# haan6/fm-for-online-recommendation

Measured on NVIDIA B200. Metric: train samples/sec (fwd+bwd+update), higher is better.
Workload: dtype f32

## Files before the change

### fm_for_online_recommendation_b200/csrc/radix_sort.cu

```cuda
#include "fmb_common.cuh"
#include "smem_sort.cuh"
#include <cooperative_groups.h>
namespace cg = cooperative_groups;

namespace {

constexpr int RADIX_BITS = 8;
constexpr int CL_SEGS = 4;
__device__ long long* g_sort_dbg = nullptr;
__device__ __forceinline__ void sort_stamp(int slot) {
    if (g_sort_dbg && threadIdx.x == 0) { unsigned long long gt; asm volatile("mov.u64 %0, %globaltimer;" : "=l"(gt)); g_sort_dbg[slot] = (long long)gt; }
}
constexpr int RADIX = 1 << RADIX_BITS;
constexpr int SORT_THREADS = 256;
constexpr int SORT_WARPS = SORT_THREADS / 32;
constexpr int KPT = 8;
constexpr int TILE = SORT_THREADS * KPT;

__device__ __forceinline__ int digit_of(int32_t key, int shift) { return (key >> shift) & (RADIX - 1); }

using fmb::digit_peers;

__global__ void __launch_bounds__(SORT_THREADS) radix_hist_kernel(const int32_t* __restrict__ keys, int64_t N,
                                                                  int shift, int ntiles,
                                                                  uint32_t* __restrict__ hist) {
    __shared__ uint32_t h[RADIX];
    for (int i = threadIdx.x; i < RADIX; i += SORT_THREADS) h[i] = 0;
    __syncthreads();
    const int64_t base = (int64_t)blockIdx.x * TILE;
#pragma unroll
    for (int i = 0; i < KPT; ++i) {
        const int64_t idx = base + (int64_t)i * SORT_THREADS + threadIdx.x;
        if (idx < N) atomicAdd(&h[digit_of(keys[idx], shift)], 1u);
    }
    __syncthreads();
    for (int i = threadIdx.x; i < RADIX; i += SORT_THREADS) hist[(size_t)i * ntiles + blockIdx.x] = h[i];
}

__global__ void __launch_bounds__(256) radix_scan_rows_kernel(uint32_t* __restrict__ hist, int ntiles, uint32_t* __restrict__ rowtot) {
    __shared__ uint32_t warp_tot[8];
    __shared__ uint32_t carry_s;
    const int lane = threadIdx.x & 31, warp = threadIdx.x >> 5;
    uint32_t* row = hist + (size_t)blockIdx.x * ntiles;
    if (threadIdx.x == 0) carry_s = 0;
    __syncthreads();
    constexpr int IPT = 4;
    for (int base = 0; base < ntiles; base += 256 * IPT) {
        const int i0 = base + threadIdx.x * IPT;
        uint32_t v[IPT], sum = 0;
#pragma unroll
        for (int j = 0; j < IPT; ++j) { v[j] = (i0 + j < ntiles) ? row[i0 + j] : 0u; sum += v[j]; }
        uint32_t inc = sum;
#pragma unroll
        for (int o = 1; o < 32; o <<= 1) { uint32_t t = __shfl_up_sync(0xffffffffu, inc, o); if (lane >= o) inc += t; }
        if (lane == 31) warp_tot[warp] = inc;
        __syncthreads();
        uint32_t before = 0, all = 0;
#pragma unroll
        for (int w = 0; w < 8; ++w) { const uint32_t t = warp_tot[w]; if (w < warp) before += t; all += t; }
        const uint32_t carry = carry_s;
        uint32_t excl = carry + before + (inc - sum);
#pragma unroll
        for (int j = 0; j < IPT; ++j) { if (i0 + j < ntiles) row[i0 + j] = excl; excl += v[j]; }
        __syncthreads();
        if (threadIdx.x == 0) carry_s = carry + all;
        __syncthreads();
    }
    if (threadIdx.x == 0) rowtot[blockIdx.x] = carry_s;
}

__global__ void __launch_bounds__(SORT_THREADS) radix_scatter_kernel(const int32_t* __restrict__ keys_in,
                                                                     const int32_t* __restrict__ vals_in, int64_t N,
                                                                     int shift, int ntiles,
                                                                     const uint32_t* __restrict__ scan,
                                                                     const uint32_t* __restrict__ rowtot,
                                                                     int32_t* __restrict__ keys_out,
                                                                     int32_t* __restrict__ vals_out) {
    __shared__ uint32_t cnt[SORT_WARPS][RADIX];
    __shared__ uint32_t gbase[RADIX];
    const int lane = threadIdx.x & 31, warp = threadIdx.x >> 5;
    for (int i = threadIdx.x; i < SORT_WARPS * RADIX; i += SORT_THREADS) (&cnt[0][0])[i] = 0;
    for (int i = threadIdx.x; i < RADIX; i += SORT_THREADS) gbase[i] = scan[(size_t)i * ntiles + blockIdx.x];
    __syncthreads();
    if (warp == 0) {
        uint32_t v[8], sum = 0;
#pragma unroll
        for (int j = 0; j < 8; ++j) { v[j] = rowtot[lane * 8 + j]; sum += v[j]; }
        uint32_t inc = sum;
#pragma unroll
        for (int o = 1; o < 32; o <<= 1) { const uint32_t t = __shfl_up_sync(0xffffffffu, inc, o); if (lane >= o) inc += t; }
        uint32_t ex = inc - sum;
#pragma unroll
        for (int j = 0; j < 8; ++j) { gbase[lane * 8 + j] += ex; ex += v[j]; }
    }
    __syncthreads();
    const int64_t wbase = (int64_t)blockIdx.x * TILE + (int64_t)warp * 32 * KPT;
    int32_t key[KPT];
    uint32_t rank[KPT];
    const uint32_t lt = (1u << lane) - 1u;
#pragma unroll
    for (int i = 0; i < KPT; ++i) {
        const int64_t idx = wbase + i * 32 + lane;
        const bool valid = idx < N;
        key[i] = valid ? keys_in[idx] : 0;
        const unsigned d = valid ? (unsigned)digit_of(key[i], shift) : 0u;
        const unsigned m = digit_peers(d, valid);
        const int leader = __ffs(m) - 1;
        uint32_t old = 0;
        if (valid && lane == leader) { old = cnt[warp][d]; cnt[warp][d] = old + __popc(m); }
        old = __shfl_sync(0xffffffffu, old, leader);
        rank[i] = old + __popc(m & lt);
        __syncwarp();
    }
    __syncthreads();
    for (int d = threadIdx.x; d < RADIX; d += SORT_THREADS) {
        uint32_t run = 0;
#pragma unroll
        for (int w = 0; w < SORT_WARPS; ++w) { uint32_t t = cnt[w][d]; cnt[w][d] = run; run += t; }
    }
    __syncthreads();
#pragma unroll
    for (int i = 0; i < KPT; ++i) {
        const int64_t idx = wbase + i * 32 + lane;
        if (idx < N) {
            const int d = digit_of(key[i], shift);
            const uint32_t pos = gbase[d] + cnt[warp][d] + rank[i];
            keys_out[pos] = key[i];
            vals_out[pos] = vals_in ? vals_in[idx] : (int32_t)idx;
        }
    }
}

__global__ void __launch_bounds__(1024) segment_starts_kernel(const int32_t* __restrict__ keys, int64_t N,
                                                              int32_t* __restrict__ seg_start,
                                                              int32_t* __restrict__ nseg) {
    __shared__ uint32_t warp_tot[32];
    __shared__ uint32_t carry_s;
    const int lane = threadIdx.x & 31, warp = threadIdx.x >> 5;
    if (threadIdx.x == 0) carry_s = 0;
    __syncthreads();
    for (int64_t base = 0; base < N; base += 1024) {
        const int64_t i = base + threadIdx.x;
        const uint32_t f = (i < N) && (i == 0 || keys[i] != keys[i - 1]);
        uint32_t inc = f;
#pragma unroll
        for (int o = 1; o < 32; o <<= 1) { uint32_t t = __shfl_up_sync(0xffffffffu, inc, o); if (lane >= o) inc += t; }
        if (lane == 31) warp_tot[warp] = inc;
        __syncthreads();
        if (warp == 0) {
            uint32_t w = warp_tot[lane], winc = w;
#pragma unroll
            for (int o = 1; o < 32; o <<= 1) { uint32_t t = __shfl_up_sync(0xffffffffu, winc, o); if (lane >= o) winc += t; }
            warp_tot[lane] = winc - w;
        }
        __syncthreads();
        const uint32_t pos = carry_s + warp_tot[warp] + inc - f;
        if (f) seg_start[pos] = (int32_t)i;
        __syncthreads();
        if (threadIdx.x == 1023) carry_s = pos + f;
        __syncthreads();
    }
    if (threadIdx.x == 0) { *nseg = (int32_t)carry_s; seg_start[carry_s] = (int32_t)N; }
}



template <int THREADS, typename KeyAt>
__device__ __forceinline__ void sort_tail(const uint32_t* kc, const uint16_t* pc, int n, int g0, int B, int F, int f,
                                          int32_t off, int32_t* __restrict__ skeys, int32_t* __restrict__ perm,
                                          uint32_t* __restrict__ posflag, int4* __restrict__ rl_entries,
                                          uint32_t* __restrict__ rl_segc, int rl_cap, int rl_nseg, int seg, int seg_long, KeyAt key_at) {
    __shared__ uint32_t wcount_s[32], wcountl_s[32];
    const int lane = threadIdx.x & 31, warp = threadIdx.x >> 5;
    const uint32_t lt = (1u << lane) - 1u;
    const int nr = (n + 31) & ~31;
    int4* mine = rl_entries ? rl_entries + (size_t)seg * rl_cap : nullptr;
    int4* minel = rl_entries ? rl_entries + (size_t)seg_long * rl_cap : nullptr;
    auto is_long = [&](int i, uint32_t key) {
        const int g2 = g0 + i + 127, j2 = i + 127;
        return g2 < B && (j2 < n ? kc[j2] : key_at(g2)) == key;
    };
    uint32_t wc = 0, wcl = 0;
    for (int i = threadIdx.x; i < nr; i += THREADS) {
        bool start = false, lng = false;
        if (i < n) {
            const int gi = g0 + i;
            const uint32_t key = kc[i];
            const uint32_t prev = gi > 0 ? (i > 0 ? kc[i - 1] : key_at(gi - 1)) : 0xffffffffu;
            const uint32_t next = gi + 1 < B ? (i + 1 < n ? kc[i + 1] : key_at(gi + 1)) : 0xffffffffu;
            const bool cont = key == prev, multi = cont || key == next;
            start = multi && !cont;
            if (start && mine) lng = is_long(i, key);
            const size_t o = (size_t)f * B + gi;
            const int32_t e = (int32_t)pc[i] * F + f;
            skeys[o] = (int32_t)key + off;
            perm[o] = e;
            if (posflag) posflag[e] = (uint32_t)o | (multi ? 0x80000000u : 0u);
        }
        if (mine) {
            wc += __popc(__ballot_sync(0xffffffffu, start && !lng));
            wcl += __popc(__ballot_sync(0xffffffffu, lng));
        }
    }
    if (!mine) return;
    if (lane == 0) { wcount_s[warp] = wc; wcountl_s[warp] = wcl; }
    __syncthreads();
    uint32_t base = 0, total = 0, basel = 0, totall = 0;
    for (int w = 0; w < THREADS / 32; ++w) {
        const uint32_t t = wcount_s[w], tl = wcountl_s[w];
        if (w < warp) { base += t; basel += tl; }
        total += t; totall += tl;
    }
    if (threadIdx.x == 0) { rl_segc[seg] = total; rl_segc[rl_nseg + seg_long] = totall; }
    if (wc + wcl == 0) return;
    for (int i = threadIdx.x; i < nr; i += THREADS) {
        uint32_t key = 0xfffffffeu;
        bool cont = false, start = false, lng = false;
        const int gi = g0 + i;
        if (i < n) {
            key = kc[i];
            const uint32_t prev = gi > 0 ? (i > 0 ? kc[i - 1] : key_at(gi - 1)) : 0xffffffffu;
            const uint32_t next = gi + 1 < B ? (i + 1 < n ? kc[i + 1] : key_at(gi + 1)) : 0xffffffffu;
            cont = key == prev;
            start = !cont && key == next;
            if (start) lng = is_long(i, key);
        }
        const unsigned m = __ballot_sync(0xffffffffu, start);
        if (m) {
            const unsigned ml = __ballot_sync(0xffffffffu, lng);
            const unsigned cm = __ballot_sync(0xffffffffu, cont);
            const uint32_t klast = __shfl_sync(0xffffffffu, key, 31);
            const int i2 = i + 32, gi2 = gi + 32;
            const uint32_t k2 = gi2 < B ? (i2 < n ? kc[i2] : key_at(gi2)) : 0xffffffffu;
            const unsigned em = __ballot_sync(0xffffffffu, k2 == klast);
            const int ext = em == 0xffffffffu ? 32 : __ffs(~em) - 1;
            if (start) {
                const unsigned after = lane == 31 ? 0u : (cm >> (lane + 1));
                const int inw = lane == 31 ? 0 : __ffs(~after) - 1;
                int n0 = 1 + inw;
                if (lane + inw == 31) n0 += ext;
                if (n0 > 32) n0 = 32;
                const int4 e4 = make_int4((int)((size_t)f * B + gi), (int32_t)key + off, n0, lng ? 1 : 0);
                if (lng) minel[rl_cap - 1 - (int)(basel + __popc(ml & lt))] = e4;
                else mine[base + __popc((m & ~ml) & lt)] = e4;
            }
            base += __popc(m & ~ml);
            basel += __popc(ml);
        }
    }
}

constexpr int SPARSE_THREADS = 1024;
constexpr int SPARSE_DIRECT = 256;

__host__ __device__ inline int sparse_table_slots(int B) { int t = 1024; while (t < 2 * B) t <<= 1; return t; }
__host__ __device__ inline size_t sparse_region_bytes(int B) {
    const size_t a = (size_t)sparse_table_slots(B) * 4, b = (size_t)B * 4 + (size_t)(B + (B & 1)) * 2 + 32 * 256 * 2;
    return a > b ? a : b;
}
__host__ __device__ inline int sparse_bp(int B) { return B < 2048 ? 2048 : B; }
__host__ __device__ inline size_t sparse_smem_bytes(int B) {
    return (size_t)B * 4 + (size_t)((B + 3) & ~3) + (size_t)sparse_bp(B) * 4 + (size_t)((sparse_bp(B) + 1) & ~1) * 2 + sparse_region_bytes(B) + 16;
}

__global__ void __launch_bounds__(SPARSE_THREADS) sparse_fields_kernel(const int32_t* __restrict__ ids, int B, int F,
                                                                      const int32_t* __restrict__ field_off,
                                                                      int64_t min_rows, int32_t* __restrict__ skeys,
                                                                      int32_t* __restrict__ perm, uint32_t* __restrict__ posflag,
                                                                      int4* __restrict__ rl_entries, uint32_t* __restrict__ rl_segc,
                                                                      int rl_cap) {
    const int f = blockIdx.x;
    const int32_t off = field_off[f];
    const uint32_t nrows = (uint32_t)(field_off[f + 1] - off);
    if ((int64_t)nrows < min_rows) return;
    extern __shared__ __align__(16) unsigned char sp_smem[];
    const int slots = sparse_table_slots(B);
    uint32_t* keys = reinterpret_cast<uint32_t*>(sp_smem);
    uint8_t* flag = reinterpret_cast<uint8_t*>(keys + B);
    const int Bp = sparse_bp(B);
    uint32_t* kbuf0 = reinterpret_cast<uint32_t*>(flag + ((B + 3) & ~3));
    uint16_t* pbuf0 = reinterpret_cast<uint16_t*>(kbuf0 + Bp);
    uint32_t* tab = reinterpret_cast<uint32_t*>(pbuf0 + ((Bp + 1) & ~1));
    uint32_t* kbuf1 = tab;
    uint16_t* pbuf1 = reinterpret_cast<uint16_t*>(kbuf1 + B);
    uint16_t* cnt = pbuf1 + B + (B & 1);
    __shared__ uint32_t tot[256];
    __shared__ uint32_t wsum[32];
    __shared__ uint32_t nm_s, t_fill, t_filll;
    const int lane = threadIdx.x & 31, warp = threadIdx.x >> 5;
    const uint32_t lt = (1u << lane) - 1u;
    sort_stamp(16 + 2 * F + 2 * f);
    for (int i0 = threadIdx.x; i0 < B; i0 += 8 * SPARSE_THREADS) {
        int32_t v[8];
#pragma unroll
        for (int u = 0; u < 8; ++u) { const int i = i0 + u * SPARSE_THREADS; v[u] = i < B ? __ldg(ids + (size_t)i * F + f) : 0; }
#pragma unroll
        for (int u = 0; u < 8; ++u) {
            const int i = i0 + u * SPARSE_THREADS;
            if (i < B) { keys[i] = (uint32_t)(v[u] - off); flag[i] = 0; }
        }
    }
    for (int i = threadIdx.x; i < slots; i += SPARSE_THREADS) tab[i] = 0;
    if (threadIdx.x == 0) { t_fill = 0; t_filll = 0; }
    __syncthreads();
    sort_stamp(16 + 6 * F + f);
    {
        constexpr int PER = 8;
        const uint32_t mask = (uint32_t)slots - 1u;
        const int hshift = 32 - (31 - __clz(slots));
        uint32_t key[PER], slot[PER], step[PER];
        unsigned open = 0;
#pragma unroll
        for (int u = 0; u < PER; ++u) {
            const int i = threadIdx.x + u * SPARSE_THREADS;
            key[u] = 0; slot[u] = 0; step[u] = 1;
            if (i < B) {
                key[u] = keys[i];
                slot[u] = (key[u] * 2654435761u) >> hshift;
                step[u] = ((key[u] * 0x85ebca6bu) >> 17) | 1u;
                open |= 1u << u;
            }
        }
#pragma unroll
        for (int u = 0; u < PER; ++u)
            if ((open >> u) & 1u) { if (tab[slot[u]] == 0u) tab[slot[u]] = (uint32_t)(threadIdx.x + u * SPARSE_THREADS) + 1u; }
        __syncthreads();
        const int perb = (B + SPARSE_THREADS - 1) / SPARSE_THREADS;
        uint16_t* ulist = reinterpret_cast<uint16_t*>(kbuf0) + warp * (perb * 32);
        uint16_t* uslot = ulist + SPARSE_THREADS * perb;
        int wn = 0;
#pragma unroll
        for (int u = 0; u < PER; ++u) {
            bool unsettled = false;
            const uint32_t me = (uint32_t)(threadIdx.x + u * SPARSE_THREADS) + 1u;
            if ((open >> u) & 1u) {
                const uint32_t cur = tab[slot[u]];
                if (cur == me) { }
                else if (keys[cur - 1] == key[u]) { flag[cur - 1] = 1; flag[me - 1] = 1; }
                else unsettled = true;
            }
            const unsigned um = __ballot_sync(0xffffffffu, unsettled);
            if (unsettled) {
                const int j = wn + __popc(um & lt);
                ulist[j] = (uint16_t)(me - 1u);
                uslot[j] = (uint16_t)((slot[u] + step[u]) & mask);
            }
            wn += __popc(um);
        }
        __syncthreads();
        for (int j = lane; j < wn; j += 32) {
            const uint32_t i = ulist[j], k = keys[i];
            const uint32_t st = ((k * 0x85ebca6bu) >> 17) | 1u;
            uint32_t sl = uslot[j];
            for (;;) {
                const uint32_t old = atomicCAS(&tab[sl], 0u, i + 1u);
                if (old == 0u) break;
                if (keys[old - 1] == k) { flag[old - 1] = 1; flag[i] = 1; break; }
                sl = (sl + st) & mask;
            }
        }
    }
    __syncthreads();
    sort_stamp(16 + 7 * F + f);
    const int per = (B + SPARSE_THREADS - 1) / SPARSE_THREADS;
    const int i0 = threadIdx.x * per;
    uint32_t mine = 0;
    for (int u = 0; u < per; ++u) if (i0 + u < B) mine += flag[i0 + u];
    uint32_t inc = mine;
#pragma unroll
    for (int o = 1; o < 32; o <<= 1) { const uint32_t t = __shfl_up_sync(0xffffffffu, inc, o); if (lane >= o) inc += t; }
    if (lane == 31) wsum[warp] = inc;
    __syncthreads();
    if (warp == 0) {
        const uint32_t w = wsum[lane];
        uint32_t winc = w;
#pragma unroll
        for (int o = 1; o < 32; o <<= 1) { const uint32_t t = __shfl_up_sync(0xffffffffu, winc, o); if (lane >= o) winc += t; }
        wsum[lane] = winc - w;
        if (lane == 31) nm_s = winc;
    }
    __syncthreads();
    {
        uint32_t o = wsum[warp] + inc - mine;
        for (int u = 0; u < per; ++u)
            if (i0 + u < B && flag[i0 + u]) { kbuf0[o] = keys[i0 + u]; pbuf0[o] = (uint16_t)(i0 + u); ++o; }
    }
    __syncthreads();
    const int nm = (int)nm_s;
    sort_stamp(16 + 5 * F + f);
    uint32_t* ks = kbuf1;
    uint16_t* ps = pbuf1;
    if (nm <= SPARSE_DIRECT) {
        for (int a = threadIdx.x; a < nm; a += SPARSE_THREADS) {
            const uint32_t key = kbuf0[a];
            int r = 0;
            for (int b2 = 0; b2 < nm; ++b2) { const uint32_t kb = kbuf0[b2]; r += (kb < key) || (kb == key && b2 < a); }
            kbuf1[r] = key;
            pbuf1[r] = pbuf0[a];
        }
        __syncthreads();
    } else {
        const int bits = nrows <= 1 ? 0 : 32 - __clz(nrows - 1);
        fmb::smem_sort_passes(kbuf0, kbuf1, pbuf0, pbuf1, cnt, tot, nm, (bits + RADIX_BITS - 1) / RADIX_BITS, &ks, &ps);
    }
    sort_stamp(16 + 8 * F + f);
    const size_t fb = (size_t)f * B;
    for (int i = nm + threadIdx.x; i < B; i += SPARSE_THREADS) skeys[fb + i] = -1;
    int4* seg = rl_entries ? rl_entries + (size_t)(f * CL_SEGS) * rl_cap : nullptr;
    const int nr = (nm + 31) & ~31;
    for (int a = threadIdx.x; a < nr; a += SPARSE_THREADS) {
        bool start = false;
        uint32_t key = 0;
        if (a < nm) {
            key = ks[a];
            const int32_t e = (int32_t)ps[a] * F + f;
            skeys[fb + a] = (int32_t)key + off;
            perm[fb + a] = e;
            posflag[e] = (uint32_t)(fb + a) | 0x80000000u;
            start = a == 0 || ks[a - 1] != key;
        }
        if (seg && start) {
            int n0 = 1;
            while (n0 < 32 && a + n0 < nm && ks[a + n0] == key) ++n0;
            const bool lng = a + 127 < nm && ks[a + 127] == key;
            const int4 e4 = make_int4((int)(fb + a), (int32_t)key + off, n0, lng ? 1 : 0);
            if (lng) seg[CL_SEGS * rl_cap - 1 - (int)atomicAdd(&t_filll, 1u)] = e4;
            else seg[atomicAdd(&t_fill, 1u)] = e4;
        }
    }
    if (seg) {
        __syncthreads();
        if (threadIdx.x < CL_SEGS) {
            rl_segc[f * CL_SEGS + threadIdx.x] = threadIdx.x == 0 ? t_fill : 0u;
            rl_segc[F * CL_SEGS + f * CL_SEGS + threadIdx.x] = threadIdx.x == CL_SEGS - 1 ? t_filll : 0u;
        }
    }
    sort_stamp(17 + 2 * F + 2 * f);
}

constexpr int FS_THREADS = 1024;
constexpr int FS_WARPS = FS_THREADS / 32;
constexpr int FS_MAX_SLOTS = 16;

__global__ void __launch_bounds__(FS_THREADS) sort_fields_kernel(const int32_t* __restrict__ ids, int B, int F,
                                                                 const int32_t* __restrict__ field_off,
                                                                 int32_t* __restrict__ skeys,
                                                                 int32_t* __restrict__ perm, uint32_t* __restrict__ posflag,
                                                                 int4* __restrict__ rl_entries, uint32_t* __restrict__ rl_segc,
                                                                 int rl_cap, int64_t max_rows) {
    extern __shared__ __align__(16) unsigned char fs_smem[];
    uint32_t* kbuf0 = reinterpret_cast<uint32_t*>(fs_smem);
    uint32_t* kbuf1 = kbuf0 + B;
    uint16_t* pbuf0 = reinterpret_cast<uint16_t*>(kbuf1 + B);
    uint16_t* pbuf1 = pbuf0 + B + (B & 1);
    uint16_t* cnt = pbuf1 + B + (B & 1);
    __shared__ uint32_t tot[RADIX];
    const int f = blockIdx.x, lane = threadIdx.x & 31, warp = threadIdx.x >> 5;
    const int32_t off = field_off[f];
    const uint32_t nrows = (uint32_t)(field_off[f + 1] - off);
    if ((int64_t)nrows >= max_rows) return;
    const int bits = nrows <= 1 ? 0 : 32 - __clz(nrows - 1);
    const int passes = (bits + RADIX_BITS - 1) / RADIX_BITS;
    (void)lane; (void)warp;
    for (int i = threadIdx.x; i < B; i += FS_THREADS) {
        kbuf0[i] = (uint32_t)(ids[(size_t)i * F + f] - off);
        pbuf0[i] = (uint16_t)i;
    }
    __syncthreads();
    uint32_t* kc; uint16_t* pc;
    fmb::smem_sort_passes(kbuf0, kbuf1, pbuf0, pbuf1, cnt, tot, B, passes, &kc, &pc);
    sort_tail<FS_THREADS>(kc, pc, B, 0, B, F, f, off, skeys, perm, posflag, rl_entries, rl_segc, rl_cap, F * CL_SEGS, f * CL_SEGS,
                          f * CL_SEGS + CL_SEGS - 1, [](int) { return 0xffffffffu; });
    if (rl_entries && threadIdx.x >= 1 && threadIdx.x < CL_SEGS) {
        rl_segc[f * CL_SEGS + threadIdx.x] = 0u;
        rl_segc[F * CL_SEGS + f * CL_SEGS + threadIdx.x - 1] = 0u;
    }
}


constexpr int CL = CL_SEGS;
#define SORT_PROBE(slot) do { if (dbg && threadIdx.x == 0) { long long t_ = clock64(); dbg[slot] += t_ - tlast; tlast = t_; } } while (0)

template <int THREADS, bool STAGED, int MAXS>
__global__ void __cluster_dims__(CL, 1, 1) __launch_bounds__(THREADS, THREADS == 256 && MAXS == 8 ? 3 : 1)
sort_fields_cluster_kernel(const int32_t* __restrict__ ids, int B, int F, const int32_t* __restrict__ field_off,
                           int32_t* __restrict__ skeys, int32_t* __restrict__ perm, int Bq, uint32_t* __restrict__ posflag,
                           int4* __restrict__ rl_entries, uint32_t* __restrict__ rl_segc, int rl_cap, int64_t max_rows) {
    constexpr int WARPS = THREADS / 32;
    extern __shared__ __align__(16) unsigned char fs_smem[];
    uint32_t* kbuf0 = reinterpret_cast<uint32_t*>(fs_smem);
    uint32_t* kbuf1 = kbuf0 + Bq;
    uint16_t* pbuf0 = reinterpret_cast<uint16_t*>(kbuf1 + Bq);
    uint16_t* pbuf1 = pbuf0 + Bq + (Bq & 1);
    uint16_t* cnt = pbuf1 + Bq + (Bq & 1);
    uint32_t* kstage = reinterpret_cast<uint32_t*>(cnt + 32 * RADIX);
    uint16_t* pstage = reinterpret_cast<uint16_t*>(kstage + Bq);
    __shared__ uint32_t lstart[RADIX];
    __shared__ uint32_t tot[RADIX];
    __shared__ uint32_t before_s[RADIX];
    __shared__ uint32_t base[RADIX];
    cg::cluster_group cluster = cg::this_cluster();
    const int crank = (int)cluster.block_rank();
    const int f = blockIdx.x / CL, lane = threadIdx.x & 31, warp = threadIdx.x >> 5;
    const int32_t off = field_off[f];
    const uint32_t nrows = (uint32_t)(field_off[f + 1] - off);
    if ((int64_t)nrows >= max_rows) return;
    const int bits = nrows <= 1 ? 0 : 32 - __clz(nrows - 1);
    const int passes = (bits + RADIX_BITS - 1) / RADIX_BITS;
    const int g0 = crank * Bq;
    const int n = max(0, min(Bq, B - g0));
    long long* dbg = (g_sort_dbg && blockIdx.x == (unsigned)(F - 1) * CL) ? g_sort_dbg : nullptr;
    long long tlast = clock64();
    if (crank == 0) sort_stamp(16 + 2 * f);
    if (g_sort_dbg && threadIdx.x == 0) {
        unsigned long long gt; asm volatile("mov.u64 %0, %globaltimer;" : "=l"(gt));
        atomicMin(reinterpret_cast<unsigned long long*>(g_sort_dbg) + 14, gt);
    }
    for (int i0 = threadIdx.x; i0 < n; i0 += 8 * THREADS) {
        int32_t v[8];
#pragma unroll
        for (int u = 0; u < 8; ++u) { const int i = i0 + u * THREADS; v[u] = i < n ? __ldg(ids + (size_t)(g0 + i) * F + f) : 0; }
#pragma unroll
        for (int u = 0; u < 8; ++u) {
            const int i = i0 + u * THREADS;
            if (i < n) { kbuf0[i] = (uint32_t)(v[u] - off); pbuf0[i] = (uint16_t)(g0 + i); }
        }
    }
    __syncthreads();
    SORT_PROBE(0);
    uint32_t* kc = kbuf0; uint32_t* kn = kbuf1;
    uint16_t* pc = pbuf0; uint16_t* pn = pbuf1;
    const int slots = (Bq + THREADS - 1) / THREADS;
    const int wbase = warp * slots * 32;
    const uint32_t lt = (1u << lane) - 1u;
    for (int ps = 0; ps < passes; ++ps) {
        const int shift = ps * RADIX_BITS;
        for (int i = threadIdx.x; i < WARPS * RADIX / 2; i += THREADS) reinterpret_cast<uint32_t*>(cnt)[i] = 0;
        __syncthreads();
        uint32_t key[MAXS];
        uint16_t rank[MAXS];
        unsigned peers[MAXS];
#pragma unroll
        for (int s = 0; s < MAXS; ++s) {
            if (s < slots) {
                const int idx = wbase + s * 32 + lane;
                const bool valid = idx < n;
                key[s] = valid ? kc[idx] : 0u;
                peers[s] = digit_peers(valid ? ((key[s] >> shift) & (RADIX - 1)) : 0u, valid);
            }
        }
#pragma unroll
        for (int s = 0; s < MAXS; ++s) {
            if (s < slots) {
                const int idx = wbase + s * 32 + lane;
                const bool valid = idx < n;
                const unsigned d = (key[s] >> shift) & (RADIX - 1);
                const unsigned m = peers[s];
                const int leader = __ffs(m) - 1;
                uint32_t old = 0;
                if (valid && lane == leader) { old = cnt[warp * RADIX + d]; cnt[warp * RADIX + d] = (uint16_t)(old + __popc(m)); }
                old = __shfl_sync(0xffffffffu, old, leader);
                rank[s] = (uint16_t)(old + __popc(m & lt));
                __syncwarp();
            }
        }
        __syncthreads();
        SORT_PROBE(1);
        if (threadIdx.x < RADIX) {
            const int d = threadIdx.x;
            uint32_t run = 0;
            for (int w = 0; w < WARPS; ++w) { const uint32_t t = cnt[w * RADIX + d]; cnt[w * RADIX + d] = (uint16_t)run; run += t; }
            tot[d] = run;
        }
        if (STAGED) {
            __syncthreads();
            SORT_PROBE(2);
            if (warp == 0) {
                uint32_t v[8], sum = 0;
#pragma unroll
                for (int j = 0; j < 8; ++j) { v[j] = tot[lane * 8 + j]; sum += v[j]; }
                uint32_t inc = sum;
#pragma unroll
                for (int o = 1; o < 32; o <<= 1) { const uint32_t t = __shfl_up_sync(0xffffffffu, inc, o); if (lane >= o) inc += t; }
                uint32_t ex = inc - sum;
#pragma unroll
                for (int j = 0; j < 8; ++j) { lstart[lane * 8 + j] = ex; ex += v[j]; }
            }
            __syncthreads();
#pragma unroll
            for (int s = 0; s < MAXS; ++s) {
                if (s < slots) {
                    const int idx = wbase + s * 32 + lane;
                    if (idx < n) {
                        const unsigned d = (key[s] >> shift) & (RADIX - 1);
                        const uint32_t lp = lstart[d] + cnt[warp * RADIX + d] + rank[s];
                        kstage[lp] = key[s];
                        pstage[lp] = pc[idx];
                    }
                }
            }
        }
        SORT_PROBE(3);
        cluster.sync();
        SORT_PROBE(4);
        if (threadIdx.x < RADIX) {
            const int d = threadIdx.x;
            uint32_t all = 0, before = 0;
#pragma unroll
            for (int r = 0; r < CL; ++r) {
                const uint32_t t = *cluster.map_shared_rank(&tot[d], r);
                all += t;
                if (r < crank) before += t;
            }
            base[d] = all;
            before_s[d] = before;
        }
        __syncthreads();
        if (warp == 0) {
            uint32_t v[8], sum = 0;
#pragma unroll
            for (int j = 0; j < 8; ++j) { v[j] = base[lane * 8 + j]; sum += v[j]; }
            uint32_t inc = sum;
#pragma unroll
            for (int o = 1; o < 32; o <<= 1) { const uint32_t t = __shfl_up_sync(0xffffffffu, inc, o); if (lane >= o) inc += t; }
            uint32_t ex = inc - sum;
#pragma unroll
            for (int j = 0; j < 8; ++j) { base[lane * 8 + j] = ex + before_s[lane * 8 + j]; ex += v[j]; }
        }
        __syncthreads();
        SORT_PROBE(5);
        if (STAGED) {
            for (int i = threadIdx.x; i < n; i += THREADS) {
                const uint32_t kk = kstage[i];
                const unsigned d = (kk >> shift) & (RADIX - 1);
                const uint32_t pos = base[d] + ((uint32_t)i - lstart[d]);
                const int dest = (pos >= (uint32_t)Bq) + (pos >= 2u * (uint32_t)Bq) + (pos >= 3u * (uint32_t)Bq);
                const uint32_t li = pos - (uint32_t)dest * (uint32_t)Bq;
                cluster.map_shared_rank(kn, dest)[li] = kk;
                cluster.map_shared_rank(pn, dest)[li] = pstage[i];
            }
        } else {
#pragma unroll
            for (int s = 0; s < MAXS; ++s) {
                if (s < slots) {
                    const int idx = wbase + s * 32 + lane;
                    if (idx < n) {
                        const unsigned d = (key[s] >> shift) & (RADIX - 1);
                        const uint32_t pos = base[d] + cnt[warp * RADIX + d] + rank[s];
                        const int dest = (pos >= (uint32_t)Bq) + (pos >= 2u * (uint32_t)Bq) + (pos >= 3u * (uint32_t)Bq);
                        const uint32_t li = pos - (uint32_t)dest * (uint32_t)Bq;
                        cluster.map_shared_rank(kn, dest)[li] = key[s];
                        cluster.map_shared_rank(pn, dest)[li] = pc[idx];
                    }
                }
            }
        }
        SORT_PROBE(6);
        cluster.sync();
        SORT_PROBE(7);
        uint32_t* tk = kc; kc = kn; kn = tk;
        uint16_t* tp = pc; pc = pn; pn = tp;
    }
    if (crank == 0) sort_stamp(16 + 4 * F + f);
    if (passes == 0) cluster.sync();
    sort_tail<THREADS>(kc, pc, n, g0, B, F, f, off, skeys, perm, posflag, rl_entries, rl_segc, rl_cap, F * CL_SEGS, f * CL_SEGS + crank, f * CL_SEGS + crank, [&](int gi) {
        const int dest = (gi >= Bq) + (gi >= 2 * Bq) + (gi >= 3 * Bq);
        return cluster.map_shared_rank(kc, dest)[gi - dest * Bq];
    });
    SORT_PROBE(8);
    cluster.sync();
    if (crank == 0) sort_stamp(17 + 2 * f);
    if (g_sort_dbg && threadIdx.x == 0) {
        unsigned long long gt; asm volatile("mov.u64 %0, %globaltimer;" : "=l"(gt));
        atomicMax(reinterpret_cast<unsigned long long*>(g_sort_dbg) + 15, gt);
        if (nrows > 100000u && crank == 0) atomicMin(reinterpret_cast<unsigned long long*>(g_sort_dbg) + 13, gt);
        if (nrows <= 256u) atomicMax(reinterpret_cast<unsigned long long*>(g_sort_dbg) + 12, gt);
    }
}

}

FMB_API void fmb_debug_set_sort_buffer(long long* dev) { cudaMemcpyToSymbol(g_sort_dbg, &dev, sizeof(dev)); }

static int sort_ntiles(int64_t N) { return (int)((N + TILE - 1) / TILE); }

FMB_API size_t fmb_sort_workspace_bytes(int64_t N) {
    const size_t n4 = ((size_t)N * 4 + 255) / 256 * 256;
    const size_t h = ((size_t)RADIX * (sort_ntiles(N) + 1) * 4 + 255) / 256 * 256;
    return 4 * n4 + h;
}

FMB_API int fmb_sort_segment(const int32_t* keys, int64_t N, int key_bits, void* ws, size_t ws_bytes,
                             int32_t* sorted_keys, int32_t* perm, int32_t* seg_start, int32_t* nseg,
                             cudaStream_t stream) {
    FMB_CHECK_ARG(keys && sorted_keys && perm && ws, "fmb_sort_segment: null pointer");
    FMB_CHECK_ARG(N > 0 && N < ((int64_t)1 << 31), "fmb_sort_segment: N out of range");
    FMB_CHECK_ARG(key_bits >= 1 && key_bits <= 31, "fmb_sort_segment: key_bits out of range");
    if (ws_bytes < fmb_sort_workspace_bytes(N)) { fmb_set_error("fmb_sort_segment: workspace too small"); return FMB_ERR_WS; }
    const size_t n4 = ((size_t)N * 4 + 255) / 256 * 256;
    char* w = (char*)ws;
    int32_t* kbuf[2] = {(int32_t*)w, (int32_t*)(w + n4)};
    int32_t* vbuf[2] = {(int32_t*)(w + 2 * n4), (int32_t*)(w + 3 * n4)};
    uint32_t* hist = (uint32_t*)(w + 4 * n4);
    const int ntiles = sort_ntiles(N);
    const int passes = (key_bits + RADIX_BITS - 1) / RADIX_BITS;
    const int32_t* kin = keys;
    const int32_t* vin = nullptr;
    for (int p = 0; p < passes; ++p) {
        const bool last = (p == passes - 1);
        int32_t* kout = last ? sorted_keys : kbuf[p & 1];
        int32_t* vout = last ? perm : vbuf[p & 1];
        const int shift = p * RADIX_BITS;
        radix_hist_kernel<<<ntiles, SORT_THREADS, 0, stream>>>(kin, N, shift, ntiles, hist);
        radix_scan_rows_kernel<<<RADIX, 256, 0, stream>>>(hist, ntiles, hist + (size_t)RADIX * ntiles);
        radix_scatter_kernel<<<ntiles, SORT_THREADS, 0, stream>>>(kin, vin, N, shift, ntiles, hist, hist + (size_t)RADIX * ntiles, kout, vout);
        kin = kout;
        vin = vout;
    }
    FMB_CHECK_LAUNCH("radix sort");
    if (seg_start) {
        FMB_CHECK_ARG(nseg, "fmb_sort_segment: seg_start given without nseg");
        segment_starts_kernel<<<1, 1024, 0, stream>>>(sorted_keys, N, seg_start, nseg);
        FMB_CHECK_LAUNCH("segment_starts_kernel");
    }
    return FMB_OK;
}

FMB_API int fmb_sort_fields_kernel_fns(const void** fns, int* nparams, int* skeys_arg) {
    fns[0] = (const void*)sort_fields_kernel; nparams[0] = 11; skeys_arg[0] = 4;
    fns[1] = (const void*)sort_fields_cluster_kernel<256, true, 16>; nparams[1] = 12; skeys_arg[1] = 4;
    fns[2] = (const void*)sort_fields_cluster_kernel<1024, false, 16>; nparams[2] = 12; skeys_arg[2] = 4;
    fns[3] = (const void*)sparse_fields_kernel; nparams[3] = 11; skeys_arg[3] = 5;
    fns[4] = (const void*)sort_fields_cluster_kernel<256, true, 8>; nparams[4] = 12; skeys_arg[4] = 4;
    return 5;
}

FMB_API int fmb_sort_fields_max_batch(void) { return 65536; }

struct fmb_runlist_t { int32_t* entries; uint32_t* seg_count; int nseg, seg_cap; };
#define FMB_SORT_SPARSE_OK 1

FMB_API void fmb_runlist_shape(int B, int F, int* nseg, int* seg_cap) {
    int Bq = (B + CL - 1) / CL;
    Bq = (Bq + 31) / 32 * 32;
    *nseg = F * CL_SEGS;
    *seg_cap = Bq;
}

FMB_API int64_t fmb_sort_fields_sparse_min_rows(int B) {
    return (B > 0 && sparse_smem_bytes(B) <= 200 * 1024) ? (int64_t)16 * B : 0;
}

#define FMB_SORT_PART_DENSE 2
#define FMB_SORT_PART_SPARSE 4
FMB_API int fmb_sort_fields_ex(const int32_t* ids, int B, int F, const int32_t* field_off, int32_t* sorted_keys,
                               int32_t* perm, uint32_t* posflag, const fmb_runlist_t* rl, int flags, cudaStream_t stream) {
    FMB_CHECK_ARG(ids && field_off && sorted_keys && perm, "fmb_sort_fields: null pointer");
    FMB_CHECK_ARG(B > 0 && B <= fmb_sort_fields_max_batch() && F > 0, "fmb_sort_fields: B=%d out of range", B);
    int Bq = (B + CL - 1) / CL;
    Bq = (Bq + 31) / 32 * 32;
    FMB_CHECK_ARG(!rl || (rl->entries && rl->seg_count && rl->nseg == F * CL_SEGS && rl->seg_cap >= Bq && F * CL_SEGS <= 2048),
                  "fmb_sort_fields: run list shape must be that of fmb_runlist_shape");
    int4* rle = rl ? reinterpret_cast<int4*>(rl->entries) : nullptr;
    uint32_t* rlc = rl ? rl->seg_count : nullptr;
    const int rcap = rl ? rl->seg_cap : 0;
    static bool attr = false;
    if (!attr) {
        cudaFuncSetAttribute(sort_fields_kernel, cudaFuncAttributeMaxDynamicSharedMemorySize, 220 * 1024);
        cudaFuncSetAttribute(sort_fields_cluster_kernel<256, true, 8>, cudaFuncAttributeMaxDynamicSharedMemorySize, 220 * 1024);
        cudaFuncSetAttribute(sort_fields_cluster_kernel<256, true, 16>, cudaFuncAttributeMaxDynamicSharedMemorySize, 220 * 1024);
        cudaFuncSetAttribute(sort_fields_cluster_kernel<1024, false, 16>, cudaFuncAttributeMaxDynamicSharedMemorySize, 220 * 1024);
        cudaFuncSetAttribute(sparse_fields_kernel, cudaFuncAttributeMaxDynamicSharedMemorySize, 220 * 1024);
        attr = true;
    }
    const bool sparse = (flags & FMB_SORT_SPARSE_OK) && posflag && fmb_sort_fields_sparse_min_rows(B) > 0;
    const int64_t split = sparse ? fmb_sort_fields_sparse_min_rows(B) : ((int64_t)1 << 40);
    const bool do_dense = !(flags & FMB_SORT_PART_SPARSE), do_sparse = sparse && !(flags & FMB_SORT_PART_DENSE);
    if (!do_dense) {
    } else if (B <= 2048) {
        sort_fields_kernel<<<F, FS_THREADS, fmb::smem_sort_bytes(B), stream>>>(ids, B, F, field_off, sorted_keys, perm, posflag,
                                                                               rle, rlc, rcap, split);
        FMB_CHECK_LAUNCH("sort_fields_kernel");
    } else {
        if (Bq <= 256 * 8)
            sort_fields_cluster_kernel<256, true, 8><<<F * CL, 256, fmb::smem_sort_bytes(Bq) + (size_t)Bq * 6 + 16, stream>>>(
                ids, B, F, field_off, sorted_keys, perm, Bq, posflag, rle, rlc, rcap, split);
        else if (Bq <= 256 * FS_MAX_SLOTS)
            sort_fields_cluster_kernel<256, true, 16><<<F * CL, 256, fmb::smem_sort_bytes(Bq) + (size_t)Bq * 6 + 16, stream>>>(
                ids, B, F, field_off, sorted_keys, perm, Bq, posflag, rle, rlc, rcap, split);
        else
            sort_fields_cluster_kernel<1024, false, 16><<<F * CL, 1024, fmb::smem_sort_bytes(Bq), stream>>>(
                ids, B, F, field_off, sorted_keys, perm, Bq, posflag, rle, rlc, rcap, split);
        FMB_CHECK_LAUNCH("sort_fields_cluster_kernel");
    }
    if (do_sparse) {
        sparse_fields_kernel<<<F, SPARSE_THREADS, sparse_smem_bytes(B), stream>>>(ids, B, F, field_off, split, sorted_keys, perm,
                                                                                   posflag, rle, rlc, rcap);
        FMB_CHECK_LAUNCH("sparse_fields_kernel");
    }
    return FMB_OK;
}

FMB_API int fmb_sort_fields(const int32_t* ids, int B, int F, const int32_t* field_off, int32_t* sorted_keys,
                            int32_t* perm, cudaStream_t stream) {
    return fmb_sort_fields_ex(ids, B, F, field_off, sorted_keys, perm, nullptr, nullptr, 0, stream);
}
```

### fm_for_online_recommendation_b200/csrc/session.cu

```cuda
#include "fmb_common.cuh"
#include <cstdlib>
#include <cstring>
#include <cstddef>
#include <new>

extern "C" {
int fmb_fm_forward(const int32_t*, const float*, const float*, const float*, int, int, int, float*, float*, float*,
                   float*, float*, const float*, int, float*, float*, cudaStream_t);
size_t fmb_sort_workspace_bytes(int64_t);
int fmb_sort_segment(const int32_t*, int64_t, int, void*, size_t, int32_t*, int32_t*, int32_t*, int32_t*,
                     cudaStream_t);
size_t fmb_bwd_workspace_bytes(int64_t, int);
int fmb_sort_fields_max_batch(void);
struct fmb_runlist_t { int32_t* entries; uint32_t* seg_count; int nseg, seg_cap; };
void fmb_runlist_shape(int, int, int*, int*);
int fmb_sort_fields_ex(const int32_t*, int, int, const int32_t*, int32_t*, int32_t*, uint32_t*, const fmb_runlist_t*, int, cudaStream_t);
int fmb_pos_flags_ex(const int32_t*, const int32_t*, int64_t, uint32_t*, const fmb_runlist_t*, cudaStream_t);
int fmb_fm_backward_update(const int32_t*, const int32_t*, int64_t, const float*, float*, int, int, const float*,
                           const float*, int, const float*, float, int, void*, size_t, cudaStream_t);
int fmb_finish_step(const float*, const float*, int, float*, float, int, float*, cudaStream_t);
struct fmb_ftrl_t { float* zn; float* bias_zn; float beta, l1, l2; };
int fmb_fm_backward_runs_list(const int32_t*, int64_t, float*, int, int, float, int, const fmb_ftrl_t*, const fmb_runlist_t*,
                              void*, size_t, cudaStream_t);
int fmb_finish_step_ex(const float*, const float*, int, float*, float, int, const fmb_ftrl_t*, float*, cudaStream_t);
int fmb_fm_step_fused_ex(const int32_t*, const float*, const float*, float*, const float*, const uint32_t*, int, int, int,
                         int, float, int, const fmb_ftrl_t*, float*, float*, void*, size_t, cudaStream_t);
int fmb_fm_backward_runs_ex(const int32_t*, int64_t, float*, int, int, float, int, const fmb_ftrl_t*, void*, size_t,
                            cudaStream_t);
int fmb_pos_flags(const int32_t*, const int32_t*, int64_t, uint32_t*, cudaStream_t);
int fmb_fm_step_fused(const int32_t*, const float*, const float*, float*, const float*, const uint32_t*, int, int, int,
                      int, float, int, float*, float*, void*, size_t, cudaStream_t);
int fmb_fm_backward_runs(const int32_t*, int64_t, float*, int, int, float, int, void*, size_t, cudaStream_t);
int fmb_is_fused_kernel_fn(const void*);
void fmb_runs_list_next_is_dependent(int);
const void* fmb_finish_kernel_fn(void);
int fmb_sort_fields_kernel_fns(const void**, int*, int*);
}

#define FMB_GRAPH_CACHE 32
struct StepVariant {
    int B, key_bits, loss_kind, mode, has_xv, pre, has_next, cur;
    const void *table, *bias;
    float lr;
    cudaGraph_t graph;
    cudaGraphExec_t exec;
    cudaGraphNode_t n_fused, n_finish, n_sort_cur[2], n_sort_next[2];
    int np_sort_cur[2], np_sort_next[2];
    int nlaunch;
    const void *cur_ids, *cur_xv, *cur_y, *cur_sort_ids, *cur_next_ids, *cur_loss;
};

struct fmb_session {
    int F, k, rowp, kp4;
    int64_t maxB;
    int32_t* d_ids;
    float* d_xv;
    float* d_y;
    float* d_S;
    float* d_z;
    float* d_delta;
    float* d_lossv;
    float* d_loss;
    int32_t* d_skeys;
    int32_t* d_perm;
    int32_t* d_skeys_buf[2];
    int32_t* d_perm_buf[2];
    uint32_t* d_posflag_buf[2];
    int32_t* d_runlist_buf[2];
    uint32_t* d_runcount_buf[2];
    int rl_nseg, rl_cap;
    void* d_sort_ws2;
    const int32_t* presort_ids;
    int presort_B, presort_buf, last_buf;
    int presort_ext;
    int presort_stale;
    cudaEvent_t ev_presort, ev_buf_free[2];
    int buf_used[2];
    void* d_sort_ws;
    size_t sort_ws_bytes;
    void* d_bwd_ws;
    size_t bwd_ws_bytes;
    int32_t* d_field_off;
    int32_t* h_ids;
    float* h_xv;
    float* h_y;
    float* h_loss;
    int32_t* d_ids2; float* d_xv2; float* d_y2; float* d_loss2;
    int32_t* h_ids2; float* h_xv2; float* h_y2;
    int32_t* d_idsx[2]; float* d_xvx[2]; float* d_yx[2];
    int32_t* h_idsx[2]; float* h_xvx[2]; float* h_yx[2];
    cudaStream_t st_copy;
    cudaEvent_t ev_h2d[4], ev_done[4];
    int slot_used[4];
    int64_t launches;
    cudaStream_t st0, st1, st2, st3, st4;
    cudaEvent_t ev_sp_fork, ev_sp_join, ev_join4;
    int64_t steps_done;
    cudaEvent_t ev_fork, ev_fwd, ev_sort, ev_join;
    int use_graph, use_prio;
    int host_path;
    int use_pdl;
    int sort_after;
    int sparse_ok;
    int ngraphs, next_evict;
    StepVariant gvar[FMB_GRAPH_CACHE];
    cudaEvent_t ev_join2;
    struct { const int32_t* ids; int B, key_bits, buf, nl; cudaGraphExec_t exec; cudaGraph_t graph; } psg[8];
    int npsg, presort_warm;
    fmb_ftrl_t ftrl;
    int ftrl_set;
};

#define CU(call)                                                                              \
    do {                                                                                      \
        cudaError_t e__ = (call);                                                             \
        if (e__ != cudaSuccess) { fmb_set_error("%s: %s", #call, cudaGetErrorString(e__)); return FMB_ERR_CUDA; } \
    } while (0)

FMB_API void fmb_session_destroy(fmb_session* s) {
    if (!s) return;
    cudaFree(s->d_ids); cudaFree(s->d_xv); cudaFree(s->d_y); cudaFree(s->d_S); cudaFree(s->d_z);
    cudaFree(s->d_delta); cudaFree(s->d_lossv); cudaFree(s->d_loss);
    for (int i = 0; i < 2; ++i) { cudaFree(s->d_skeys_buf[i]); cudaFree(s->d_perm_buf[i]); cudaFree(s->d_posflag_buf[i]); cudaFree(s->d_runlist_buf[i]); cudaFree(s->d_runcount_buf[i]); if (s->ev_buf_free[i]) cudaEventDestroy(s->ev_buf_free[i]); }
    cudaFree(s->d_sort_ws2);
    if (s->ev_join2) cudaEventDestroy(s->ev_join2);
    for (int i = 0; i < s->npsg; ++i) if (s->psg[i].exec) { cudaGraphExecDestroy(s->psg[i].exec); cudaGraphDestroy(s->psg[i].graph); }
    if (s->ev_sp_fork) cudaEventDestroy(s->ev_sp_fork);
    if (s->ev_sp_join) cudaEventDestroy(s->ev_sp_join);
    if (s->st3) cudaStreamDestroy(s->st3);
    if (s->st4) cudaStreamDestroy(s->st4);
    if (s->ev_join4) cudaEventDestroy(s->ev_join4);
    if (s->ev_presort) cudaEventDestroy(s->ev_presort);
    cudaFree(s->d_sort_ws); cudaFree(s->d_bwd_ws); cudaFree(s->d_field_off);
    cudaFreeHost(s->h_ids); cudaFreeHost(s->h_xv); cudaFreeHost(s->h_y); cudaFreeHost(s->h_loss);
    cudaFree(s->d_ids2); cudaFree(s->d_xv2); cudaFree(s->d_y2); cudaFree(s->d_loss2);
    cudaFreeHost(s->h_ids2); cudaFreeHost(s->h_xv2); cudaFreeHost(s->h_y2);
    if (s->st_copy) cudaStreamDestroy(s->st_copy);
    for (int i = 0; i < 4; ++i) { if (s->ev_h2d[i]) cudaEventDestroy(s->ev_h2d[i]); if (s->ev_done[i]) cudaEventDestroy(s->ev_done[i]); }
    for (int i = 0; i < 2; ++i) {
        cudaFree(s->d_idsx[i]); cudaFree(s->d_xvx[i]); cudaFree(s->d_yx[i]);
        cudaFreeHost(s->h_idsx[i]); cudaFreeHost(s->h_xvx[i]); cudaFreeHost(s->h_yx[i]);
    }
    for (int i = 0; i < s->ngraphs; ++i) { cudaGraphExecDestroy(s->gvar[i].exec); cudaGraphDestroy(s->gvar[i].graph); }
    if (s->st0) cudaStreamDestroy(s->st0);
    if (s->st1) cudaStreamDestroy(s->st1);
    if (s->st2) cudaStreamDestroy(s->st2);
    if (s->ev_fork) cudaEventDestroy(s->ev_fork);
    if (s->ev_fwd) cudaEventDestroy(s->ev_fwd);
    if (s->ev_sort) cudaEventDestroy(s->ev_sort);
    if (s->ev_join) cudaEventDestroy(s->ev_join);
    delete s;
}

FMB_API int fmb_session_create(fmb_session** out, int F, int k, int64_t max_batch, const int32_t* field_off_host) {
    FMB_CHECK_ARG(out && F > 0 && k > 0 && max_batch > 0, "fmb_session_create: bad arguments");
    FMB_CHECK_ARG(max_batch * F < ((int64_t)1 << 31), "fmb_session_create: max_batch*F must fit int32");
    fmb_session* s = new (std::nothrow) fmb_session();
    FMB_CHECK_ARG(s, "fmb_session_create: out of host memory");
    memset(s, 0, sizeof(*s));
    s->F = F; s->k = k; s->rowp = fmb_round_up(k + 1, 16); s->kp4 = fmb_round_up(k, 4); s->maxB = max_batch;
    const int64_t N = max_batch * F;
    fmb_runlist_shape((int)(max_batch < 65536 ? max_batch : 65536), F, &s->rl_nseg, &s->rl_cap);
    if ((int64_t)s->rl_nseg * s->rl_cap < N / 2 + 64) s->rl_cap = (int)((N / 2 + 64 + s->rl_nseg - 1) / s->rl_nseg);
    s->sort_ws_bytes = fmb_sort_workspace_bytes(N);
    s->bwd_ws_bytes = fmb_bwd_workspace_bytes(N, k);
    cudaError_t e = cudaSuccess;
    auto dm = [&](void** p, size_t n) { if (e == cudaSuccess) e = cudaMalloc(p, n); };
    auto hm = [&](void** p, size_t n) { if (e == cudaSuccess) e = cudaMallocHost(p, n); };
    dm((void**)&s->d_ids, N * 4); dm((void**)&s->d_xv, N * 4); dm((void**)&s->d_y, max_batch * 4);
    dm((void**)&s->d_S, max_batch * s->kp4 * 4); dm((void**)&s->d_z, max_batch * 4);
    dm((void**)&s->d_delta, max_batch * 4); dm((void**)&s->d_lossv, max_batch * 4); dm((void**)&s->d_loss, 256);
    for (int i = 0; i < 2; ++i) { dm((void**)&s->d_skeys_buf[i], N * 4); dm((void**)&s->d_perm_buf[i], N * 4); dm((void**)&s->d_posflag_buf[i], N * 4); dm((void**)&s->d_runlist_buf[i], (size_t)s->rl_nseg * s->rl_cap * 16); dm((void**)&s->d_runcount_buf[i], (size_t)s->rl_nseg * 8 + 256); }
    if (!(field_off_host && max_batch <= fmb_sort_fields_max_batch())) dm(&s->d_sort_ws2, s->sort_ws_bytes);
    s->d_skeys = s->d_skeys_buf[0]; s->d_perm = s->d_perm_buf[0];
    dm(&s->d_sort_ws, s->sort_ws_bytes); dm(&s->d_bwd_ws, s->bwd_ws_bytes);
    hm((void**)&s->h_ids, N * 4); hm((void**)&s->h_xv, N * 4); hm((void**)&s->h_y, max_batch * 4);
    hm((void**)&s->h_loss, 256);
    dm((void**)&s->d_ids2, N * 4); dm((void**)&s->d_xv2, N * 4); dm((void**)&s->d_y2, max_batch * 4);
    dm((void**)&s->d_loss2, 256);
    hm((void**)&s->h_ids2, N * 4); hm((void**)&s->h_xv2, N * 4); hm((void**)&s->h_y2, max_batch * 4);
    if (e == cudaSuccess) e = cudaStreamCreateWithFlags(&s->st_copy, cudaStreamNonBlocking);
    for (int i = 0; i < 4; ++i) {
        if (e == cudaSuccess) e = cudaEventCreateWithFlags(&s->ev_h2d[i], cudaEventDisableTiming);
        if (e == cudaSuccess) e = cudaEventCreateWithFlags(&s->ev_done[i], cudaEventDisableTiming);
    }
    if (field_off_host) {
        dm((void**)&s->d_field_off, (size_t)(F + 1) * 4);
        if (e == cudaSuccess) e = cudaMemcpy(s->d_field_off, field_off_host, (size_t)(F + 1) * 4, cudaMemcpyHostToDevice);
    }
    {
        int least = 0, greatest = 0;
        const char* pe = getenv("FMB_PRIO");
        s->use_prio = pe ? atoi(pe) : 1;
        if (s->use_prio && cudaDeviceGetStreamPriorityRange(&least, &greatest) != cudaSuccess) s->use_prio = 0;
        if (!s->use_prio) least = greatest = 0;
        if (s->use_prio == 1) { const int t = least; least = greatest; greatest = t; }
        if (e == cudaSuccess) e = cudaStreamCreateWithPriority(&s->st0, cudaStreamNonBlocking, greatest);
        if (e == cudaSuccess) e = cudaStreamCreateWithPriority(&s->st1, cudaStreamNonBlocking, greatest);
        if (e == cudaSuccess) e = cudaStreamCreateWithPriority(&s->st2, cudaStreamNonBlocking, least);
        if (e == cudaSuccess) e = cudaStreamCreateWithPriority(&s->st3, cudaStreamNonBlocking, least);
        if (e == cudaSuccess) e = cudaStreamCreateWithPriority(&s->st4, cudaStreamNonBlocking, greatest);
        if (e == cudaSuccess) e = cudaEventCreateWithFlags(&s->ev_join4, cudaEventDisableTiming);
        if (e == cudaSuccess) e = cudaEventCreateWithFlags(&s->ev_sp_fork, cudaEventDisableTiming);
        if (e == cudaSuccess) e = cudaEventCreateWithFlags(&s->ev_sp_join, cudaEventDisableTiming);
    }
    if (e == cudaSuccess) e = cudaEventCreateWithFlags(&s->ev_fork, cudaEventDisableTiming);
    if (e == cudaSuccess) e = cudaEventCreateWithFlags(&s->ev_fwd, cudaEventDisableTiming);
    if (e == cudaSuccess) e = cudaEventCreateWithFlags(&s->ev_sort, cudaEventDisableTiming);
    if (e == cudaSuccess) e = cudaEventCreateWithFlags(&s->ev_join, cudaEventDisableTiming);
    if (e == cudaSuccess) e = cudaEventCreateWithFlags(&s->ev_presort, cudaEventDisableTiming);
    if (e == cudaSuccess) e = cudaEventCreateWithFlags(&s->ev_join2, cudaEventDisableTiming);
    for (int i = 0; i < 2; ++i) if (e == cudaSuccess) e = cudaEventCreateWithFlags(&s->ev_buf_free[i], cudaEventDisableTiming);
    {
        const char* ng = getenv("FMB_NO_GRAPH");
        s->use_graph = !(ng && ng[0] == '1');
        const char* sp = getenv("FMB_SPARSE");
        s->sparse_ok = !(sp && sp[0] == '0');
        const char* pd = getenv("FMB_PDL");
        s->use_pdl = !(pd && pd[0] == '0');
        const char* sa = getenv("FMB_SORT_AFTER");
        s->sort_after = sa && sa[0] == '1';
    }
    if (e != cudaSuccess) {
        fmb_set_error("fmb_session_create: %s", cudaGetErrorString(e));
        fmb_session_destroy(s);
        return FMB_ERR_CUDA;
    }
    *out = s;
    return FMB_OK;
}

FMB_API int fmb_session_set_ftrl(fmb_session* s, float* zn_dev, float* bias_zn_dev, float beta, float l1, float l2) {
    FMB_CHECK_ARG(s && zn_dev && bias_zn_dev && l1 >= 0.f && l2 >= 0.f, "fmb_session_set_ftrl: bad arguments");
    s->ftrl.zn = zn_dev; s->ftrl.bias_zn = bias_zn_dev; s->ftrl.beta = beta; s->ftrl.l1 = l1; s->ftrl.l2 = l2;
    s->ftrl_set = 1;
    for (int i = 0; i < s->ngraphs; ++i) { cudaGraphExecDestroy(s->gvar[i].exec); cudaGraphDestroy(s->gvar[i].graph); }
    s->ngraphs = 0; s->next_evict = 0;
    return FMB_OK;
}

FMB_API int64_t fmb_session_launches(const fmb_session* s) { return s ? s->launches : 0; }
FMB_API int fmb_session_graph_count(const fmb_session* s) { return s ? s->ngraphs : 0; }

static bool by_field_sort(const fmb_session* s, int B) { return s->d_field_off && B <= fmb_sort_fields_max_batch(); }

static int sort_launch(fmb_session* s, const int32_t* ids, int B, int key_bits, int buf, void* radix_ws,
                       cudaStream_t st, int* nlaunch) {
    const int64_t N = (int64_t)B * s->F;
    int rc;
    fmb_runlist_t rl;
    rl.entries = s->d_runlist_buf[buf]; rl.seg_count = s->d_runcount_buf[buf];
    if (by_field_sort(s, B)) {
        fmb_runlist_shape(B, s->F, &rl.nseg, &rl.seg_cap);
        if (!s->sparse_ok) {
            *nlaunch += 1;
            return fmb_sort_fields_ex(ids, B, s->F, s->d_field_off, s->d_skeys_buf[buf], s->d_perm_buf[buf],
                                      s->d_posflag_buf[buf], &rl, 0, st);
        }
        cudaMemsetAsync(s->d_posflag_buf[buf], 0, (size_t)N * 4, st);
        cudaEventRecord(s->ev_sp_fork, st);
        cudaStreamWaitEvent(s->st3, s->ev_sp_fork, 0);
        rc = fmb_sort_fields_ex(ids, B, s->F, s->d_field_off, s->d_skeys_buf[buf], s->d_perm_buf[buf], s->d_posflag_buf[buf],
                                &rl, 1 | 2, st);
        if (rc) return rc;
        rc = fmb_sort_fields_ex(ids, B, s->F, s->d_field_off, s->d_skeys_buf[buf], s->d_perm_buf[buf], s->d_posflag_buf[buf],
                                &rl, 1 | 4, s->st3);
        cudaEventRecord(s->ev_sp_join, s->st3);
        cudaStreamWaitEvent(st, s->ev_sp_join, 0);
        *nlaunch += 2;
        return rc;
    } else {
        rc = fmb_sort_segment(ids, N, key_bits, radix_ws, s->sort_ws_bytes, s->d_skeys_buf[buf], s->d_perm_buf[buf],
                              nullptr, nullptr, st);
        *nlaunch += 3 * ((key_bits + 7) / 8);
    }
    if (rc) return rc;
    rl.nseg = 1; rl.seg_cap = (int)(N / 2 + 1);
    cudaMemsetAsync(s->d_runcount_buf[buf], 0, 8, st);
    rc = fmb_pos_flags_ex(s->d_skeys_buf[buf], s->d_perm_buf[buf], N, s->d_posflag_buf[buf], &rl, st);
    *nlaunch += 1;
    return rc;
}

static int fm_step_launch(fmb_session* s, const int32_t* ids, const float* xv, const float* y, int B, float* table,
                          float* bias, int key_bits, int loss_kind, float lr, int mode, float* loss_dev,
                          const int32_t* next_ids, cudaStream_t main, cudaStream_t side, cudaStream_t side2, int cur,
                          bool pre, int* nlaunch) {
    const int64_t N = (int64_t)B * s->F;
    int rc;
    *nlaunch = 0;
    cudaEventRecord(s->ev_fork, main);
    cudaStreamWaitEvent(side, s->ev_fork, 0);
    if (next_ids && !s->sort_after) {
        cudaStreamWaitEvent(side2, s->ev_fork, 0);
        rc = sort_launch(s, next_ids, B, key_bits, 1 - cur, s->d_sort_ws2, side2, nlaunch);
        if (rc) return rc;
        cudaEventRecord(s->ev_join2, side2);
    }
    if (!pre) {
        rc = sort_launch(s, ids, B, key_bits, cur, s->d_sort_ws, main, nlaunch);
        if (rc) return rc;
    }
    const fmb_ftrl_t* ft = s->ftrl_set ? &s->ftrl : nullptr;
    rc = fmb_fm_step_fused_ex(ids, xv, y, table, bias, s->d_posflag_buf[cur], B, s->F, s->k, loss_kind, lr, mode, ft,
                              s->d_delta, s->d_lossv, s->d_bwd_ws, s->bwd_ws_bytes, main);
    if (rc) return rc;
    cudaEventRecord(s->ev_fwd, main);
    cudaStreamWaitEvent(side, s->ev_fwd, 0);
    if (next_ids && s->sort_after) {
        cudaStreamWaitEvent(side2, s->ev_fwd, 0);
        rc = sort_launch(s, next_ids, B, key_bits, 1 - cur, s->d_sort_ws2, side2, nlaunch);
        if (rc) return rc;
        cudaEventRecord(s->ev_join2, side2);
    }
    rc = fmb_finish_step_ex(s->d_delta, s->d_lossv, B, bias, lr, mode, ft, loss_dev ? loss_dev : s->d_loss, side);
    if (rc) return rc;
    cudaEventRecord(s->ev_join, side);
    fmb_runlist_t rl;
    rl.entries = s->d_runlist_buf[cur]; rl.seg_count = s->d_runcount_buf[cur];
    if (by_field_sort(s, B)) fmb_runlist_shape(B, s->F, &rl.nseg, &rl.seg_cap);
    else { rl.nseg = 1; rl.seg_cap = (int)(N / 2 + 1); }
    fmb_runs_list_next_is_dependent(s->use_pdl);
    rc = fmb_fm_backward_runs_list(s->d_skeys_buf[cur], N, table, s->F, s->k, lr, mode, ft, &rl, s->d_bwd_ws, s->bwd_ws_bytes, main);
    if (rc) return rc;
    cudaStreamWaitEvent(main, s->ev_join, 0);
    if (next_ids) cudaStreamWaitEvent(main, s->ev_join2, 0);
    *nlaunch += 3;
    return FMB_OK;
}

static int patch_node(cudaGraphExec_t exec, cudaGraphNode_t node, int nparams, const void* const* repl) {
    cudaKernelNodeParams kp;
    CU(cudaGraphKernelNodeGetParams(node, &kp));
    void* args[16];
    for (int i = 0; i < nparams; ++i) args[i] = repl[i] ? const_cast<void*>(repl[i]) : kp.kernelParams[i];
    kp.kernelParams = args;
    kp.extra = nullptr;
    CU(cudaGraphExecKernelNodeSetParams(exec, node, &kp));
    return FMB_OK;
}

static int capture_variant(fmb_session* s, StepVariant* v, const int32_t* ids, const float* xv, const float* y,
                           float* table, float* bias, const int32_t* next_ids) {
    cudaGraph_t graph = nullptr;
    int nl = 0;
    CU(cudaStreamBeginCapture(s->st0, cudaStreamCaptureModeThreadLocal));
    const int rc = fm_step_launch(s, ids, xv, y, v->B, table, bias, v->key_bits, v->loss_kind, v->lr, v->mode, s->d_loss,
                                  next_ids, s->st0, s->st1, s->st2, v->cur, v->pre != 0, &nl);
    cudaError_t e = cudaStreamEndCapture(s->st0, &graph);
    if (rc) { if (graph) cudaGraphDestroy(graph); return rc; }
    if (e != cudaSuccess) { fmb_set_error("graph capture: %s", cudaGetErrorString(e)); return FMB_ERR_CUDA; }
    cudaGraphNode_t nodes[64];
    size_t nn = 64;
    CU(cudaGraphGetNodes(graph, nodes, &nn));
    const void* sort_fns[8];
    int sort_np[8], sort_ska[8];
    const int nsort = fmb_sort_fields_kernel_fns(sort_fns, sort_np, sort_ska);
    v->n_fused = v->n_finish = nullptr;
    for (int j = 0; j < 2; ++j) v->n_sort_cur[j] = v->n_sort_next[j] = nullptr;
    for (size_t i = 0; i < nn; ++i) {
        cudaGraphNodeType ty;
        CU(cudaGraphNodeGetType(nodes[i], &ty));
        if (ty != cudaGraphNodeTypeKernel) continue;
        cudaKernelNodeParams kp;
        CU(cudaGraphKernelNodeGetParams(nodes[i], &kp));
        if (fmb_is_fused_kernel_fn(kp.func)) { v->n_fused = nodes[i]; continue; }
        if (kp.func == fmb_finish_kernel_fn()) { v->n_finish = nodes[i]; continue; }
        for (int t = 0; t < nsort; ++t)
            if (kp.func == sort_fns[t]) {
                const int32_t* out = *static_cast<int32_t**>(kp.kernelParams[sort_ska[t]]);
                const bool is_cur = out == s->d_skeys_buf[v->cur];
                cudaGraphNode_t* dst = is_cur ? v->n_sort_cur : v->n_sort_next;
                int* dnp = is_cur ? v->np_sort_cur : v->np_sort_next;
                const int j = dst[0] ? 1 : 0;
                dst[j] = nodes[i]; dnp[j] = sort_np[t];
            }
    }
    if (!v->n_fused || !v->n_finish || (!v->pre && !v->n_sort_cur[0]) || (v->has_next && !v->n_sort_next[0])) {
        cudaGraphDestroy(graph);
        fmb_set_error("step graph: kernel nodes not found");
        return FMB_ERR_CUDA;
    }
    cudaGraphExec_t exec = nullptr;
    e = cudaGraphInstantiate(&exec, graph, s->use_prio ? cudaGraphInstantiateFlagUseNodePriority : 0);
    if (e != cudaSuccess) { cudaGraphDestroy(graph); fmb_set_error("graph instantiate: %s", cudaGetErrorString(e)); return FMB_ERR_CUDA; }
    v->graph = graph; v->exec = exec; v->nlaunch = nl;
    return FMB_OK;
}

FMB_API int fmb_session_fm_step_next(fmb_session* s, const int32_t* ids, const float* xv, const float* y, int B,
                                     float* table, float* bias, int key_bits, int loss_kind, float lr, int mode,
                                     const int32_t* next_ids, float* loss_dev, cudaStream_t stream) {
    FMB_CHECK_ARG(s && ids && y && table && bias, "fmb_session_fm_step: null pointer");
    FMB_CHECK_ARG(B > 0 && B <= s->maxB, "fmb_session_fm_step: B=%d exceeds session max_batch", B);
    int nl = 0;
    const bool pre = s->presort_ids == ids && s->presort_B == B && !s->presort_stale;
    s->presort_stale = 0;
    const int cur = pre ? s->presort_buf : 1 - s->last_buf;
    if (pre) {
        if (s->presort_ext) CU(cudaStreamWaitEvent(stream, s->ev_presort, 0));
    } else {
        if (s->buf_used[cur]) CU(cudaStreamWaitEvent(stream, s->ev_buf_free[cur], 0));
        if (s->presort_ids && s->presort_ext) CU(cudaStreamWaitEvent(stream, s->ev_presort, 0));
    }
    s->presort_ids = nullptr;
    if (next_ids && s->buf_used[1 - cur]) CU(cudaStreamWaitEvent(stream, s->ev_buf_free[1 - cur], 0));
    s->last_buf = cur;
    int rc = FMB_OK;
    if (!s->use_graph || s->steps_done == 0 || !by_field_sort(s, B)) {
        rc = fm_step_launch(s, ids, xv, y, B, table, bias, key_bits, loss_kind, lr, mode, loss_dev, next_ids, stream,
                            s->st1, s->st2, cur, pre, &nl);
        if (rc) return rc;
        s->launches += nl;
    } else {
        StepVariant key;
        memset(&key, 0, sizeof(key));
        key.B = B; key.key_bits = key_bits; key.loss_kind = loss_kind; key.mode = mode; key.has_xv = xv != nullptr;
        key.pre = pre; key.has_next = next_ids != nullptr; key.cur = cur; key.table = table; key.bias = bias; key.lr = lr;
        StepVariant* v = nullptr;
        const size_t keylen = offsetof(StepVariant, graph);
        float* want_loss = loss_dev ? loss_dev : s->d_loss;
        int same_key = 0;
        for (int i = 0; i < s->ngraphs; ++i)
            if (memcmp(&s->gvar[i], &key, keylen) == 0) {
                ++same_key;
                if (!v) v = &s->gvar[i];
                if (s->gvar[i].cur_ids == ids && s->gvar[i].cur_y == y && s->gvar[i].cur_loss == want_loss) { v = &s->gvar[i]; same_key = 99; break; }
            }
        if (v && same_key < 4 && s->host_path) v = nullptr;
        if (!v) {
            rc = capture_variant(s, &key, ids, xv, y, table, bias, next_ids);
            if (rc) return rc;
            int slot;
            if (s->ngraphs < FMB_GRAPH_CACHE) slot = s->ngraphs++;
            else {
                slot = s->next_evict; s->next_evict = (s->next_evict + 1) % FMB_GRAPH_CACHE;
                cudaGraphExecDestroy(s->gvar[slot].exec); cudaGraphDestroy(s->gvar[slot].graph);
            }
            s->gvar[slot] = key;
            v = &s->gvar[slot];
        }
        if (v->cur_ids != ids || v->cur_xv != xv || v->cur_y != y) {
            const void* repl[16] = {nullptr};
            repl[0] = &ids; repl[1] = &xv; repl[2] = &y;
            rc = patch_node(v->exec, v->n_fused, 5, repl);
            if (rc) return rc;
            v->cur_ids = ids; v->cur_xv = xv; v->cur_y = y;
        }
        if (!pre && v->cur_sort_ids != ids) {
            const void* repl[16] = {nullptr};
            repl[0] = &ids;
            for (int j = 0; j < 2 && v->n_sort_cur[j]; ++j) {
                rc = patch_node(v->exec, v->n_sort_cur[j], v->np_sort_cur[j], repl);
                if (rc) return rc;
            }
            v->cur_sort_ids = ids;
        }
        if (next_ids && v->cur_next_ids != next_ids) {
            const void* repl[16] = {nullptr};
            repl[0] = &next_ids;
            for (int j = 0; j < 2 && v->n_sort_next[j]; ++j) {
                rc = patch_node(v->exec, v->n_sort_next[j], v->np_sort_next[j], repl);
                if (rc) return rc;
            }
            v->cur_next_ids = next_ids;
        }
        {
            float* lo = loss_dev ? loss_dev : s->d_loss;
            if (v->cur_loss != lo) {
                const void* repl[16] = {nullptr};
                repl[6] = &lo;
                rc = patch_node(v->exec, v->n_finish, 9, repl);
                if (rc) return rc;
                v->cur_loss = lo;
            }
        }
        CU(cudaGraphLaunch(v->exec, stream));
        s->launches += v->nlaunch;
    }
    CU(cudaEventRecord(s->ev_buf_free[cur], stream));
    s->buf_used[cur] = 1;
    if (next_ids) {
        s->presort_ids = next_ids; s->presort_B = B; s->presort_buf = 1 - cur; s->presort_ext = 0;
        CU(cudaEventRecord(s->ev_buf_free[1 - cur], stream));
        s->buf_used[1 - cur] = 1;
    }
    s->steps_done += 1;
    return FMB_OK;
}

FMB_API int fmb_session_fm_step(fmb_session* s, const int32_t* ids, const float* xv, const float* y, int B,
                                float* table, float* bias, int key_bits, int loss_kind, float lr, int mode,
                                float* loss_dev, cudaStream_t stream) {
    return fmb_session_fm_step_next(s, ids, xv, y, B, table, bias, key_bits, loss_kind, lr, mode, nullptr, loss_dev, stream);
}

static int presort_impl(fmb_session* s, const int32_t* ids, int B, int key_bits, cudaEvent_t ready) {
    const int buf = 1 - s->last_buf;
    if (s->buf_used[buf]) CU(cudaStreamWaitEvent(s->st2, s->ev_buf_free[buf], 0));
    if (ready) CU(cudaStreamWaitEvent(s->st2, ready, 0));
    int nl = 0;
    if (s->use_graph && s->presort_warm && by_field_sort(s, B)) {
        int g = -1;
        for (int i = 0; i < s->npsg; ++i)
            if (s->psg[i].ids == ids && s->psg[i].B == B && s->psg[i].key_bits == key_bits && s->psg[i].buf == buf) g = i;
        if (g < 0) {
            cudaGraph_t graph = nullptr;
            CU(cudaStreamBeginCapture(s->st2, cudaStreamCaptureModeThreadLocal));
            const int rc = sort_launch(s, ids, B, key_bits, buf, s->d_sort_ws2 ? s->d_sort_ws2 : s->d_sort_ws, s->st2, &nl);
            const cudaError_t e = cudaStreamEndCapture(s->st2, &graph);
            if (rc) { if (graph) cudaGraphDestroy(graph); return rc; }
            if (e != cudaSuccess) { fmb_set_error("pre-sort graph capture: %s", cudaGetErrorString(e)); return FMB_ERR_CUDA; }
            cudaGraphExec_t exec = nullptr;
            if (cudaGraphInstantiate(&exec, graph, 0) != cudaSuccess) { cudaGraphDestroy(graph); fmb_set_error("pre-sort graph instantiate failed"); return FMB_ERR_CUDA; }
            g = s->npsg < 8 ? s->npsg++ : 0;
            if (s->psg[g].exec) { cudaGraphExecDestroy(s->psg[g].exec); cudaGraphDestroy(s->psg[g].graph); }
            s->psg[g].ids = ids; s->psg[g].B = B; s->psg[g].key_bits = key_bits; s->psg[g].buf = buf; s->psg[g].nl = nl;
            s->psg[g].exec = exec; s->psg[g].graph = graph;
        }
        nl = s->psg[g].nl;
        CU(cudaGraphLaunch(s->psg[g].exec, s->st2));
    } else {
        const int rc = sort_launch(s, ids, B, key_bits, buf, s->d_sort_ws2 ? s->d_sort_ws2 : s->d_sort_ws, s->st2, &nl);
        if (rc) return rc;
        s->presort_warm = 1;
    }
    CU(cudaEventRecord(s->ev_presort, s->st2));
    s->launches += nl;
    s->presort_ids = ids; s->presort_B = B; s->presort_buf = buf; s->presort_ext = 1;
    return FMB_OK;
}

FMB_API int fmb_session_presort(fmb_session* s, const int32_t* ids, int B, int key_bits) {
    FMB_CHECK_ARG(s && ids && B > 0 && B <= s->maxB, "fmb_session_presort: bad arguments");
    return presort_impl(s, ids, B, key_bits, nullptr);
}

FMB_API void fmb_session_presort_invalidate(fmb_session* s) {
    if (!s || !s->presort_ids) return;
    s->presort_stale = 1;
}

static bool host_ptr_is_pinned(const void* p) {
    static thread_local const void* seen[16];
    static thread_local bool pinned[16];
    static thread_local int nseen = 0, nextw = 0;
    for (int i = 0; i < nseen; ++i) if (seen[i] == p) return pinned[i];
    cudaPointerAttributes a;
    bool r = false;
    if (cudaPointerGetAttributes(&a, p) != cudaSuccess) cudaGetLastError();
    else r = a.type == cudaMemoryTypeHost;
    seen[nextw] = p; pinned[nextw] = r; nextw = (nextw + 1) % 16; if (nseen < 16) ++nseen;
    return r;
}
FMB_API int fmb_session_fm_step_host_async(fmb_session* s, int slot, const int32_t* ids_host, const float* xv_host,
                                           const float* y_host, int B, float* table, float* bias, int key_bits,
                                           int loss_kind, float lr, int mode, cudaStream_t stream) {
    FMB_CHECK_ARG(s && ids_host && y_host && table && bias, "fmb_session_fm_step_host_async: null pointer");
    FMB_CHECK_ARG(slot >= 0 && slot < 4, "fmb_session_fm_step_host_async: slot must be 0..3");
    FMB_CHECK_ARG(B > 0 && B <= s->maxB, "fmb_session_fm_step_host_async: B=%d exceeds session max_batch", B);
    const size_t N = (size_t)B * s->F;
    if (slot >= 2 && !s->d_idsx[slot - 2]) {
        const size_t NN = (size_t)s->maxB * s->F;
        const int j = slot - 2;
        cudaError_t e = cudaMalloc((void**)&s->d_idsx[j], NN * 4);
        if (e == cudaSuccess) e = cudaMalloc((void**)&s->d_xvx[j], NN * 4);
        if (e == cudaSuccess) e = cudaMalloc((void**)&s->d_yx[j], (size_t)s->maxB * 4);
        if (e == cudaSuccess) e = cudaMallocHost((void**)&s->h_idsx[j], NN * 4);
        if (e == cudaSuccess) e = cudaMallocHost((void**)&s->h_xvx[j], NN * 4);
        if (e == cudaSuccess) e = cudaMallocHost((void**)&s->h_yx[j], (size_t)s->maxB * 4);
        if (e != cudaSuccess) { fmb_set_error("fmb_session_fm_step_host_async: %s", cudaGetErrorString(e)); return FMB_ERR_CUDA; }
    }
    int32_t* d_ids = slot >= 2 ? s->d_idsx[slot - 2] : (slot ? s->d_ids2 : s->d_ids);
    float* d_xv = slot >= 2 ? s->d_xvx[slot - 2] : (slot ? s->d_xv2 : s->d_xv);
    float* d_y = slot >= 2 ? s->d_yx[slot - 2] : (slot ? s->d_y2 : s->d_y);
    float* d_loss = slot ? s->d_loss2 : s->d_loss;
    int32_t* h_ids = slot >= 2 ? s->h_idsx[slot - 2] : (slot ? s->h_ids2 : s->h_ids);
    float* h_xv = slot >= 2 ? s->h_xvx[slot - 2] : (slot ? s->h_xv2 : s->h_xv);
    float* h_y = slot >= 2 ? s->h_yx[slot - 2] : (slot ? s->h_y2 : s->h_y);
    if (s->slot_used[slot]) CU(cudaEventSynchronize(s->ev_done[slot]));
    const void* src_ids = ids_host;
    const void* src_y = y_host;
    const void* src_xv = xv_host;
    if (!host_ptr_is_pinned(ids_host)) { memcpy(h_ids, ids_host, N * 4); src_ids = h_ids; }
    if (!host_ptr_is_pinned(y_host)) { memcpy(h_y, y_host, (size_t)B * 4); src_y = h_y; }
    if (xv_host && !host_ptr_is_pinned(xv_host)) { memcpy(h_xv, xv_host, N * 4); src_xv = h_xv; }
    CU(cudaMemcpyAsync(d_ids, src_ids, N * 4, cudaMemcpyHostToDevice, s->st_copy));
    CU(cudaMemcpyAsync(d_y, src_y, (size_t)B * 4, cudaMemcpyHostToDevice, s->st_copy));
    if (xv_host) CU(cudaMemcpyAsync(d_xv, src_xv, N * 4, cudaMemcpyHostToDevice, s->st_copy));
    CU(cudaEventRecord(s->ev_h2d[slot], s->st_copy));
    CU(cudaStreamWaitEvent(stream, s->ev_h2d[slot], 0));
    int rc = presort_impl(s, d_ids, B, key_bits, s->ev_h2d[slot]);
    if (rc) return rc;
    (void)d_loss;
    s->host_path = 1;
    rc = fmb_session_fm_step(s, d_ids, xv_host ? d_xv : nullptr, d_y, B, table, bias, key_bits, loss_kind, lr,
                                 mode, s->h_loss + 8 * slot, stream);
    s->host_path = 0;
    if (rc) return rc;
    CU(cudaEventRecord(s->ev_done[slot], stream));
    s->slot_used[slot] = 1;
    return FMB_OK;
}

FMB_API int fmb_session_host_slots(void) { return 4; }

FMB_API int fmb_session_wait_loss(fmb_session* s, int slot, float* loss_host) {
    FMB_CHECK_ARG(s && slot >= 0 && slot < 4 && s->slot_used[slot], "fmb_session_wait_loss: nothing submitted on slot %d", slot);
    CU(cudaEventSynchronize(s->ev_done[slot]));
    if (loss_host) *loss_host = s->h_loss[8 * slot];
    return FMB_OK;
}

FMB_API int fmb_session_fm_step_host(fmb_session* s, const int32_t* ids_host, const float* xv_host,
                                     const float* y_host, int B, float* table, float* bias, int key_bits,
                                     int loss_kind, float lr, int mode, float* loss_host, cudaStream_t stream) {
    FMB_CHECK_ARG(s && ids_host && y_host && table && bias, "fmb_session_fm_step_host: null pointer");
    FMB_CHECK_ARG(B > 0 && B <= s->maxB, "fmb_session_fm_step_host: B=%d exceeds session max_batch", B);
    const size_t N = (size_t)B * s->F;
    memcpy(s->h_ids, ids_host, N * 4);
    memcpy(s->h_y, y_host, (size_t)B * 4);
    CU(cudaMemcpyAsync(s->d_ids, s->h_ids, N * 4, cudaMemcpyHostToDevice, stream));
    CU(cudaMemcpyAsync(s->d_y, s->h_y, (size_t)B * 4, cudaMemcpyHostToDevice, stream));
    if (xv_host) {
        memcpy(s->h_xv, xv_host, N * 4);
        CU(cudaMemcpyAsync(s->d_xv, s->h_xv, N * 4, cudaMemcpyHostToDevice, stream));
    }
    int rc = fmb_session_fm_step(s, s->d_ids, xv_host ? s->d_xv : nullptr, s->d_y, B, table, bias, key_bits,
                                 loss_kind, lr, mode, s->d_loss, stream);
    if (rc) return rc;
    CU(cudaMemcpyAsync(s->h_loss, s->d_loss, 4, cudaMemcpyDeviceToHost, stream));
    CU(cudaStreamSynchronize(stream));
    if (loss_host) *loss_host = s->h_loss[0];
    return FMB_OK;
}
```

Baseline: 202.6 million.

## Replace split dense/sparse field sort with a single cluster step sort kernel

```diff
diff --git a/fm_for_online_recommendation_b200/csrc/radix_sort.cu b/fm_for_online_recommendation_b200/csrc/radix_sort.cu
--- a/fm_for_online_recommendation_b200/csrc/radix_sort.cu
+++ b/fm_for_online_recommendation_b200/csrc/radix_sort.cu
@@ -8,8 +8,12 @@
 constexpr int RADIX_BITS = 8;
 constexpr int CL_SEGS = 4;
 __device__ long long* g_sort_dbg = nullptr;
+__device__ __forceinline__ long long* sort_dbg() { return *reinterpret_cast<long long* volatile*>(&g_sort_dbg); }
 __device__ __forceinline__ void sort_stamp(int slot) {
-    if (g_sort_dbg && threadIdx.x == 0) { unsigned long long gt; asm volatile("mov.u64 %0, %globaltimer;" : "=l"(gt)); g_sort_dbg[slot] = (long long)gt; }
+    if (threadIdx.x == 0) {
+        long long* dbg = sort_dbg();
+        if (dbg) { unsigned long long gt; asm volatile("mov.u64 %0, %globaltimer;" : "=l"(gt)); dbg[slot] = (long long)gt; }
+    }
 }
 constexpr int RADIX = 1 << RADIX_BITS;
 constexpr int SORT_THREADS = 256;
@@ -166,7 +170,7 @@
 
 
 template <int THREADS, typename KeyAt>
-__device__ __forceinline__ void sort_tail(const uint32_t* kc, const uint16_t* pc, int n, int g0, int B, int F, int f,
+__device__ __forceinline__ void sort_tail(const uint32_t* kc, const uint16_t* pc, int n, int g0, int len, int B, int F, int f,
                                           int32_t off, int32_t* __restrict__ skeys, int32_t* __restrict__ perm,
                                           uint32_t* __restrict__ posflag, int4* __restrict__ rl_entries,
                                           uint32_t* __restrict__ rl_segc, int rl_cap, int rl_nseg, int seg, int seg_long, KeyAt key_at) {
@@ -178,7 +182,7 @@
     int4* minel = rl_entries ? rl_entries + (size_t)seg_long * rl_cap : nullptr;
     auto is_long = [&](int i, uint32_t key) {
         const int g2 = g0 + i + 127, j2 = i + 127;
-        return g2 < B && (j2 < n ? kc[j2] : key_at(g2)) == key;
+        return g2 < len && (j2 < n ? kc[j2] : key_at(g2)) == key;
     };
     uint32_t wc = 0, wcl = 0;
     for (int i = threadIdx.x; i < nr; i += THREADS) {
@@ -187,7 +191,7 @@
             const int gi = g0 + i;
             const uint32_t key = kc[i];
             const uint32_t prev = gi > 0 ? (i > 0 ? kc[i - 1] : key_at(gi - 1)) : 0xffffffffu;
-            const uint32_t next = gi + 1 < B ? (i + 1 < n ? kc[i + 1] : key_at(gi + 1)) : 0xffffffffu;
+            const uint32_t next = gi + 1 < len ? (i + 1 < n ? kc[i + 1] : key_at(gi + 1)) : 0xffffffffu;
             const bool cont = key == prev, multi = cont || key == next;
             start = multi && !cont;
             if (start && mine) lng = is_long(i, key);
@@ -220,7 +224,7 @@
         if (i < n) {
             key = kc[i];
             const uint32_t prev = gi > 0 ? (i > 0 ? kc[i - 1] : key_at(gi - 1)) : 0xffffffffu;
-            const uint32_t next = gi + 1 < B ? (i + 1 < n ? kc[i + 1] : key_at(gi + 1)) : 0xffffffffu;
+            const uint32_t next = gi + 1 < len ? (i + 1 < n ? kc[i + 1] : key_at(gi + 1)) : 0xffffffffu;
             cont = key == prev;
             start = !cont && key == next;
             if (start) lng = is_long(i, key);
@@ -231,7 +235,7 @@
             const unsigned cm = __ballot_sync(0xffffffffu, cont);
             const uint32_t klast = __shfl_sync(0xffffffffu, key, 31);
             const int i2 = i + 32, gi2 = gi + 32;
-            const uint32_t k2 = gi2 < B ? (i2 < n ? kc[i2] : key_at(gi2)) : 0xffffffffu;
+            const uint32_t k2 = gi2 < len ? (i2 < n ? kc[i2] : key_at(gi2)) : 0xffffffffu;
             const unsigned em = __ballot_sync(0xffffffffu, k2 == klast);
             const int ext = em == 0xffffffffu ? 32 : __ffs(~em) - 1;
             if (start) {
@@ -250,194 +254,6 @@
     }
 }
 
-constexpr int SPARSE_THREADS = 1024;
-constexpr int SPARSE_DIRECT = 256;
-
-__host__ __device__ inline int sparse_table_slots(int B) { int t = 1024; while (t < 2 * B) t <<= 1; return t; }
-__host__ __device__ inline size_t sparse_region_bytes(int B) {
-    const size_t a = (size_t)sparse_table_slots(B) * 4, b = (size_t)B * 4 + (size_t)(B + (B & 1)) * 2 + 32 * 256 * 2;
-    return a > b ? a : b;
-}
-__host__ __device__ inline int sparse_bp(int B) { return B < 2048 ? 2048 : B; }
-__host__ __device__ inline size_t sparse_smem_bytes(int B) {
-    return (size_t)B * 4 + (size_t)((B + 3) & ~3) + (size_t)sparse_bp(B) * 4 + (size_t)((sparse_bp(B) + 1) & ~1) * 2 + sparse_region_bytes(B) + 16;
-}
-
-__global__ void __launch_bounds__(SPARSE_THREADS) sparse_fields_kernel(const int32_t* __restrict__ ids, int B, int F,
-                                                                      const int32_t* __restrict__ field_off,
-                                                                      int64_t min_rows, int32_t* __restrict__ skeys,
-                                                                      int32_t* __restrict__ perm, uint32_t* __restrict__ posflag,
-                                                                      int4* __restrict__ rl_entries, uint32_t* __restrict__ rl_segc,
-                                                                      int rl_cap) {
-    const int f = blockIdx.x;
-    const int32_t off = field_off[f];
-    const uint32_t nrows = (uint32_t)(field_off[f + 1] - off);
-    if ((int64_t)nrows < min_rows) return;
-    extern __shared__ __align__(16) unsigned char sp_smem[];
-    const int slots = sparse_table_slots(B);
-    uint32_t* keys = reinterpret_cast<uint32_t*>(sp_smem);
-    uint8_t* flag = reinterpret_cast<uint8_t*>(keys + B);
-    const int Bp = sparse_bp(B);
-    uint32_t* kbuf0 = reinterpret_cast<uint32_t*>(flag + ((B + 3) & ~3));
-    uint16_t* pbuf0 = reinterpret_cast<uint16_t*>(kbuf0 + Bp);
-    uint32_t* tab = reinterpret_cast<uint32_t*>(pbuf0 + ((Bp + 1) & ~1));
-    uint32_t* kbuf1 = tab;
-    uint16_t* pbuf1 = reinterpret_cast<uint16_t*>(kbuf1 + B);
-    uint16_t* cnt = pbuf1 + B + (B & 1);
-    __shared__ uint32_t tot[256];
-    __shared__ uint32_t wsum[32];
-    __shared__ uint32_t nm_s, t_fill, t_filll;
-    const int lane = threadIdx.x & 31, warp = threadIdx.x >> 5;
-    const uint32_t lt = (1u << lane) - 1u;
-    sort_stamp(16 + 2 * F + 2 * f);
-    for (int i0 = threadIdx.x; i0 < B; i0 += 8 * SPARSE_THREADS) {
-        int32_t v[8];
-#pragma unroll
-        for (int u = 0; u < 8; ++u) { const int i = i0 + u * SPARSE_THREADS; v[u] = i < B ? __ldg(ids + (size_t)i * F + f) : 0; }
-#pragma unroll
-        for (int u = 0; u < 8; ++u) {
-            const int i = i0 + u * SPARSE_THREADS;
-            if (i < B) { keys[i] = (uint32_t)(v[u] - off); flag[i] = 0; }
-        }
-    }
-    for (int i = threadIdx.x; i < slots; i += SPARSE_THREADS) tab[i] = 0;
-    if (threadIdx.x == 0) { t_fill = 0; t_filll = 0; }
-    __syncthreads();
-    sort_stamp(16 + 6 * F + f);
-    {
-        constexpr int PER = 8;
-        const uint32_t mask = (uint32_t)slots - 1u;
-        const int hshift = 32 - (31 - __clz(slots));
-        uint32_t key[PER], slot[PER], step[PER];
-        unsigned open = 0;
-#pragma unroll
-        for (int u = 0; u < PER; ++u) {
-            const int i = threadIdx.x + u * SPARSE_THREADS;
-            key[u] = 0; slot[u] = 0; step[u] = 1;
-            if (i < B) {
-                key[u] = keys[i];
-                slot[u] = (key[u] * 2654435761u) >> hshift;
-                step[u] = ((key[u] * 0x85ebca6bu) >> 17) | 1u;
-                open |= 1u << u;
-            }
-        }
-#pragma unroll
-        for (int u = 0; u < PER; ++u)
-            if ((open >> u) & 1u) { if (tab[slot[u]] == 0u) tab[slot[u]] = (uint32_t)(threadIdx.x + u * SPARSE_THREADS) + 1u; }
-        __syncthreads();
-        const int perb = (B + SPARSE_THREADS - 1) / SPARSE_THREADS;
-        uint16_t* ulist = reinterpret_cast<uint16_t*>(kbuf0) + warp * (perb * 32);
-        uint16_t* uslot = ulist + SPARSE_THREADS * perb;
-        int wn = 0;
-#pragma unroll
-        for (int u = 0; u < PER; ++u) {
-            bool unsettled = false;
-            const uint32_t me = (uint32_t)(threadIdx.x + u * SPARSE_THREADS) + 1u;
-            if ((open >> u) & 1u) {
-                const uint32_t cur = tab[slot[u]];
-                if (cur == me) { }
-                else if (keys[cur - 1] == key[u]) { flag[cur - 1] = 1; flag[me - 1] = 1; }
-                else unsettled = true;
-            }
-            const unsigned um = __ballot_sync(0xffffffffu, unsettled);
-            if (unsettled) {
-                const int j = wn + __popc(um & lt);
-                ulist[j] = (uint16_t)(me - 1u);
-                uslot[j] = (uint16_t)((slot[u] + step[u]) & mask);
-            }
-            wn += __popc(um);
-        }
-        __syncthreads();
-        for (int j = lane; j < wn; j += 32) {
-            const uint32_t i = ulist[j], k = keys[i];
-            const uint32_t st = ((k * 0x85ebca6bu) >> 17) | 1u;
-            uint32_t sl = uslot[j];
-            for (;;) {
-                const uint32_t old = atomicCAS(&tab[sl], 0u, i + 1u);
-                if (old == 0u) break;
-                if (keys[old - 1] == k) { flag[old - 1] = 1; flag[i] = 1; break; }
-                sl = (sl + st) & mask;
-            }
-        }
-    }
-    __syncthreads();
-    sort_stamp(16 + 7 * F + f);
-    const int per = (B + SPARSE_THREADS - 1) / SPARSE_THREADS;
-    const int i0 = threadIdx.x * per;
-    uint32_t mine = 0;
-    for (int u = 0; u < per; ++u) if (i0 + u < B) mine += flag[i0 + u];
-    uint32_t inc = mine;
-#pragma unroll
-    for (int o = 1; o < 32; o <<= 1) { const uint32_t t = __shfl_up_sync(0xffffffffu, inc, o); if (lane >= o) inc += t; }
-    if (lane == 31) wsum[warp] = inc;
-    __syncthreads();
-    if (warp == 0) {
-        const uint32_t w = wsum[lane];
-        uint32_t winc = w;
-#pragma unroll
-        for (int o = 1; o < 32; o <<= 1) { const uint32_t t = __shfl_up_sync(0xffffffffu, winc, o); if (lane >= o) winc += t; }
-        wsum[lane] = winc - w;
-        if (lane == 31) nm_s = winc;
-    }
-    __syncthreads();
-    {
-        uint32_t o = wsum[warp] + inc - mine;
-        for (int u = 0; u < per; ++u)
-            if (i0 + u < B && flag[i0 + u]) { kbuf0[o] = keys[i0 + u]; pbuf0[o] = (uint16_t)(i0 + u); ++o; }
-    }
-    __syncthreads();
-    const int nm = (int)nm_s;
-    sort_stamp(16 + 5 * F + f);
-    uint32_t* ks = kbuf1;
-    uint16_t* ps = pbuf1;
-    if (nm <= SPARSE_DIRECT) {
-        for (int a = threadIdx.x; a < nm; a += SPARSE_THREADS) {
-            const uint32_t key = kbuf0[a];
-            int r = 0;
-            for (int b2 = 0; b2 < nm; ++b2) { const uint32_t kb = kbuf0[b2]; r += (kb < key) || (kb == key && b2 < a); }
-            kbuf1[r] = key;
-            pbuf1[r] = pbuf0[a];
-        }
-        __syncthreads();
-    } else {
-        const int bits = nrows <= 1 ? 0 : 32 - __clz(nrows - 1);
-        fmb::smem_sort_passes(kbuf0, kbuf1, pbuf0, pbuf1, cnt, tot, nm, (bits + RADIX_BITS - 1) / RADIX_BITS, &ks, &ps);
-    }
-    sort_stamp(16 + 8 * F + f);
-    const size_t fb = (size_t)f * B;
-    for (int i = nm + threadIdx.x; i < B; i += SPARSE_THREADS) skeys[fb + i] = -1;
-    int4* seg = rl_entries ? rl_entries + (size_t)(f * CL_SEGS) * rl_cap : nullptr;
-    const int nr = (nm + 31) & ~31;
-    for (int a = threadIdx.x; a < nr; a += SPARSE_THREADS) {
-        bool start = false;
-        uint32_t key = 0;
-        if (a < nm) {
-            key = ks[a];
-            const int32_t e = (int32_t)ps[a] * F + f;
-            skeys[fb + a] = (int32_t)key + off;
-            perm[fb + a] = e;
-            posflag[e] = (uint32_t)(fb + a) | 0x80000000u;
-            start = a == 0 || ks[a - 1] != key;
-        }
-        if (seg && start) {
-            int n0 = 1;
-            while (n0 < 32 && a + n0 < nm && ks[a + n0] == key) ++n0;
-            const bool lng = a + 127 < nm && ks[a + 127] == key;
-            const int4 e4 = make_int4((int)(fb + a), (int32_t)key + off, n0, lng ? 1 : 0);
-            if (lng) seg[CL_SEGS * rl_cap - 1 - (int)atomicAdd(&t_filll, 1u)] = e4;
-            else seg[atomicAdd(&t_fill, 1u)] = e4;
-        }
-    }
-    if (seg) {
-        __syncthreads();
-        if (threadIdx.x < CL_SEGS) {
-            rl_segc[f * CL_SEGS + threadIdx.x] = threadIdx.x == 0 ? t_fill : 0u;
-            rl_segc[F * CL_SEGS + f * CL_SEGS + threadIdx.x] = threadIdx.x == CL_SEGS - 1 ? t_filll : 0u;
-        }
-    }
-    sort_stamp(17 + 2 * F + 2 * f);
-}
-
 constexpr int FS_THREADS = 1024;
 constexpr int FS_WARPS = FS_THREADS / 32;
 constexpr int FS_MAX_SLOTS = 16;
@@ -447,7 +263,7 @@
                                                                  int32_t* __restrict__ skeys,
                                                                  int32_t* __restrict__ perm, uint32_t* __restrict__ posflag,
                                                                  int4* __restrict__ rl_entries, uint32_t* __restrict__ rl_segc,
-                                                                 int rl_cap, int64_t max_rows) {
+                                                                 int rl_cap) {
     extern __shared__ __align__(16) unsigned char fs_smem[];
     uint32_t* kbuf0 = reinterpret_cast<uint32_t*>(fs_smem);
     uint32_t* kbuf1 = kbuf0 + B;
@@ -458,7 +274,6 @@
     const int f = blockIdx.x, lane = threadIdx.x & 31, warp = threadIdx.x >> 5;
     const int32_t off = field_off[f];
     const uint32_t nrows = (uint32_t)(field_off[f + 1] - off);
-    if ((int64_t)nrows >= max_rows) return;
     const int bits = nrows <= 1 ? 0 : 32 - __clz(nrows - 1);
     const int passes = (bits + RADIX_BITS - 1) / RADIX_BITS;
     (void)lane; (void)warp;
@@ -469,7 +284,7 @@
     __syncthreads();
     uint32_t* kc; uint16_t* pc;
     fmb::smem_sort_passes(kbuf0, kbuf1, pbuf0, pbuf1, cnt, tot, B, passes, &kc, &pc);
-    sort_tail<FS_THREADS>(kc, pc, B, 0, B, F, f, off, skeys, perm, posflag, rl_entries, rl_segc, rl_cap, F * CL_SEGS, f * CL_SEGS,
+    sort_tail<FS_THREADS>(kc, pc, B, 0, B, B, F, f, off, skeys, perm, posflag, rl_entries, rl_segc, rl_cap, F * CL_SEGS, f * CL_SEGS,
                           f * CL_SEGS + CL_SEGS - 1, [](int) { return 0xffffffffu; });
     if (rl_entries && threadIdx.x >= 1 && threadIdx.x < CL_SEGS) {
         rl_segc[f * CL_SEGS + threadIdx.x] = 0u;
@@ -485,7 +300,7 @@
 __global__ void __cluster_dims__(CL, 1, 1) __launch_bounds__(THREADS, THREADS == 256 && MAXS == 8 ? 3 : 1)
 sort_fields_cluster_kernel(const int32_t* __restrict__ ids, int B, int F, const int32_t* __restrict__ field_off,
                            int32_t* __restrict__ skeys, int32_t* __restrict__ perm, int Bq, uint32_t* __restrict__ posflag,
-                           int4* __restrict__ rl_entries, uint32_t* __restrict__ rl_segc, int rl_cap, int64_t max_rows) {
+                           int4* __restrict__ rl_entries, uint32_t* __restrict__ rl_segc, int rl_cap) {
     constexpr int WARPS = THREADS / 32;
     extern __shared__ __align__(16) unsigned char fs_smem[];
     uint32_t* kbuf0 = reinterpret_cast<uint32_t*>(fs_smem);
@@ -504,7 +319,6 @@
     const int f = blockIdx.x / CL, lane = threadIdx.x & 31, warp = threadIdx.x >> 5;
     const int32_t off = field_off[f];
     const uint32_t nrows = (uint32_t)(field_off[f + 1] - off);
-    if ((int64_t)nrows >= max_rows) return;
     const int bits = nrows <= 1 ? 0 : 32 - __clz(nrows - 1);
     const int passes = (bits + RADIX_BITS - 1) / RADIX_BITS;
     const int g0 = crank * Bq;
@@ -663,7 +477,7 @@
     }
     if (crank == 0) sort_stamp(16 + 4 * F + f);
     if (passes == 0) cluster.sync();
-    sort_tail<THREADS>(kc, pc, n, g0, B, F, f, off, skeys, perm, posflag, rl_entries, rl_segc, rl_cap, F * CL_SEGS, f * CL_SEGS + crank, f * CL_SEGS + crank, [&](int gi) {
+    sort_tail<THREADS>(kc, pc, n, g0, B, B, F, f, off, skeys, perm, posflag, rl_entries, rl_segc, rl_cap, F * CL_SEGS, f * CL_SEGS + crank, f * CL_SEGS + crank, [&](int gi) {
         const int dest = (gi >= Bq) + (gi >= 2 * Bq) + (gi >= 3 * Bq);
         return cluster.map_shared_rank(kc, dest)[gi - dest * Bq];
     });
@@ -675,6 +489,281 @@
         atomicMax(reinterpret_cast<unsigned long long*>(g_sort_dbg) + 15, gt);
         if (nrows > 100000u && crank == 0) atomicMin(reinterpret_cast<unsigned long long*>(g_sort_dbg) + 13, gt);
         if (nrows <= 256u) atomicMax(reinterpret_cast<unsigned long long*>(g_sort_dbg) + 12, gt);
+    }
+}
+
+constexpr int ST_THREADS = 256;
+constexpr int ST_WARPS = ST_THREADS / 32;
+constexpr int ST_MAX_B = CL * 2048;
+constexpr int SPARSE_DIRECT = 256;
+static_assert(ST_THREADS == RADIX, "one thread per digit");
+
+__host__ __device__ inline int step_table_slots(int Bq) { int t = 64; while (t < 2 * Bq) t <<= 1; return t; }
+__host__ __device__ inline int step_sort_bq(int B) { return ((B + CL - 1) / CL + 31) / 32 * 32; }
+constexpr int ST_QC = ST_MAX_B / CL;
+constexpr int ST_TC = 2 * ST_QC;
+constexpr uint32_t ST_EMPTY = 0xffffffffu;
+constexpr size_t ST_HASH = (size_t)ST_TC * 5 + (size_t)ST_QC * 3;
+constexpr size_t ST_REGION = ST_HASH > (size_t)ST_QC * 8 ? ST_HASH : (size_t)ST_QC * 8;
+constexpr size_t ST_SMEM = (size_t)ST_QC * 12 + (size_t)ST_WARPS * RADIX * 2 + ST_REGION;
+
+__device__ __forceinline__ void step_sort_event(int slot, bool end) {
+    if (threadIdx.x == 0) {
+        long long* dbg = sort_dbg();
+        if (!dbg) return;
+        unsigned long long gt; asm volatile("mov.u64 %0, %globaltimer;" : "=l"(gt));
+        if (slot >= 0) dbg[slot] = (long long)gt;
+        unsigned long long* u = reinterpret_cast<unsigned long long*>(dbg);
+        if (end) atomicMax(u + 15, gt); else atomicMin(u + 14, gt);
+    }
+}
+
+__global__ void __cluster_dims__(CL, 1, 1) __launch_bounds__(ST_THREADS, 8)
+sort_fields_step_kernel(const int32_t* __restrict__ ids, int B, int F, const int32_t* __restrict__ field_off,
+                        int32_t* __restrict__ skeys, int32_t* __restrict__ perm, int64_t sparse_min, uint32_t* __restrict__ posflag,
+                        int4* __restrict__ rl_entries, uint32_t* __restrict__ rl_segc, int rl_cap) {
+    extern __shared__ __align__(16) unsigned char st_smem[];
+    __shared__ uint32_t lstart[RADIX];
+    __shared__ uint32_t tot[RADIX];
+    __shared__ uint32_t base[RADIX];
+    __shared__ uint32_t wsum[ST_WARPS];
+    __shared__ uint32_t nloc_s;
+    cg::cluster_group cluster = cg::this_cluster();
+    const int crank = (int)cluster.block_rank();
+    const int f = blockIdx.x / CL, lane = threadIdx.x & 31, warp = threadIdx.x >> 5;
+    const uint32_t lt = (1u << lane) - 1u;
+    const int32_t off = field_off[f];
+    const uint32_t nrows = (uint32_t)(field_off[f + 1] - off);
+    const bool sparse = (int64_t)nrows >= sparse_min;
+    const int Bq = step_sort_bq(B);
+    uint32_t* kA = reinterpret_cast<uint32_t*>(st_smem);
+    uint32_t* kB = kA + ST_QC;
+    uint16_t* pA = reinterpret_cast<uint16_t*>(kB + ST_QC);
+    uint16_t* pB = pA + ST_QC;
+    uint16_t* cnt = pB + ST_QC;
+    unsigned char* region = reinterpret_cast<unsigned char*>(cnt + ST_WARPS * RADIX);
+    const int g0 = crank * Bq;
+    const int n0 = max(0, min(Bq, B - g0));
+    step_sort_event(crank ? -1 : 16 + (sparse ? 2 * F : 0) + 2 * f, false);
+    for (int i0 = threadIdx.x; i0 < n0; i0 += 4 * ST_THREADS) {
+        int32_t v[4];
+#pragma unroll
+        for (int u = 0; u < 4; ++u) { const int i = i0 + u * ST_THREADS; v[u] = i < n0 ? __ldg(ids + (size_t)(g0 + i) * F + f) : 0; }
+#pragma unroll
+        for (int u = 0; u < 4; ++u) {
+            const int i = i0 + u * ST_THREADS;
+            if (i < n0) { kA[i] = (uint32_t)(v[u] - off); pA[i] = (uint16_t)(g0 + i); }
+        }
+    }
+    auto kbuf = [&](int par) { return kA + par * ST_QC; };
+    auto pbuf = [&](int par) { return pA + par * ST_QC; };
+    int cur = 0, n = n0, total = B;
+    if (sparse) {
+        const int lslots = step_table_slots(Bq), hshift = 32 - (31 - __clz(lslots));
+        const uint32_t mask = (uint32_t)lslots - 1u;
+        uint32_t* tab = reinterpret_cast<uint32_t*>(region);
+        uint8_t* mflag = region + ST_TC * 4;
+        uint16_t* eslot = reinterpret_cast<uint16_t*>(mflag + ST_TC);
+        uint8_t* flag = reinterpret_cast<uint8_t*>(eslot + ST_QC);
+        for (int i = threadIdx.x; i < lslots; i += ST_THREADS) { tab[i] = ST_EMPTY; mflag[i] = 0; }
+        __syncthreads();
+        if (crank == 0) sort_stamp(16 + 6 * F + f);
+        for (int i = threadIdx.x; i < n0; i += ST_THREADS) {
+            const uint32_t key = kA[i], step = ((key * 0x85ebca6bu) >> 17) | 1u;
+            uint32_t sl = (key * 2654435761u) >> hshift;
+            for (;;) {
+                uint32_t cur = tab[sl];
+                if (cur == ST_EMPTY) cur = atomicCAS(&tab[sl], ST_EMPTY, key);
+                if (cur == ST_EMPTY) break;
+                if (cur == key) { mflag[sl] = 1; break; }
+                sl = (sl + step) & mask;
+            }
+            eslot[i] = (uint16_t)sl;
+        }
+        cluster.sync();
+        for (int sl0 = threadIdx.x; sl0 < lslots; sl0 += ST_THREADS) {
+            const uint32_t key = tab[sl0];
+            if (key == ST_EMPTY || mflag[sl0]) continue;
+            const uint32_t step = ((key * 0x85ebca6bu) >> 17) | 1u, h = (key * 2654435761u) >> hshift;
+            for (int r = 1; r < CL && !mflag[sl0]; ++r) {
+                const uint32_t* rt = cluster.map_shared_rank(tab, (crank + r) & (CL - 1));
+                for (uint32_t sl = h;; sl = (sl + step) & mask) {
+                    const uint32_t k = rt[sl];
+                    if (k == key) { mflag[sl0] = 1; break; }
+                    if (k == ST_EMPTY) break;
+                }
+            }
+        }
+        __syncthreads();
+        for (int i = threadIdx.x; i < n0; i += ST_THREADS) flag[i] = mflag[eslot[i]];
+        __syncthreads();
+        if (crank == 0) sort_stamp(16 + 7 * F + f);
+        const int per = (n0 + ST_THREADS - 1) / ST_THREADS;
+        const int i0 = threadIdx.x * per;
+        uint32_t mine = 0;
+        for (int u = 0; u < per; ++u) if (i0 + u < n0) mine += flag[i0 + u];
+        uint32_t inc = mine;
+#pragma unroll
+        for (int o = 1; o < 32; o <<= 1) { const uint32_t t = __shfl_up_sync(0xffffffffu, inc, o); if (lane >= o) inc += t; }
+        if (lane == 31) wsum[warp] = inc;
+        __syncthreads();
+        uint32_t o = inc - mine, all = 0;
+        for (int w = 0; w < ST_WARPS; ++w) { const uint32_t t = wsum[w]; if (w < warp) o += t; all += t; }
+        for (int u = 0; u < per; ++u) {
+            const int i = i0 + u;
+            if (i >= n0) break;
+            if (flag[i]) { kB[o] = kA[i]; pB[o] = pA[i]; ++o; }
+            else posflag[(size_t)(g0 + i) * F + f] = 0u;
+        }
+        if (threadIdx.x == 0) nloc_s = all;
+        cluster.sync();
+        total = 0;
+        for (int r = 0; r < CL; ++r) total += (int)*cluster.map_shared_rank(&nloc_s, r);
+        n = (int)all;
+        cur = 1;
+        for (int i = max(g0, total) + threadIdx.x; i < g0 + n0; i += ST_THREADS) skeys[(size_t)f * B + i] = -1;
+        if (crank == 0) sort_stamp(16 + 5 * F + f);
+        if (total <= SPARSE_DIRECT) {
+            uint32_t* kall = reinterpret_cast<uint32_t*>(region);
+            uint16_t* pall = reinterpret_cast<uint16_t*>(kall + SPARSE_DIRECT);
+            int acc = 0;
+            for (int r = 0; r < CL; ++r) {
+                const int c = (int)*cluster.map_shared_rank(&nloc_s, r);
+                for (int j = threadIdx.x; j < c; j += ST_THREADS) {
+                    kall[acc + j] = cluster.map_shared_rank(kB, r)[j];
+                    pall[acc + j] = cluster.map_shared_rank(pB, r)[j];
+                }
+                acc += c;
+            }
+            __syncthreads();
+            const int Qd = ((total + CL - 1) / CL + 31) / 32 * 32, q0 = crank * Qd;
+            for (int a = threadIdx.x; a < total; a += ST_THREADS) {
+                const uint32_t key = kall[a];
+                int r = 0;
+                for (int b2 = 0; b2 < total; ++b2) { const uint32_t kb = kall[b2]; r += (kb < key) || (kb == key && b2 < a); }
+                if (r >= q0 && r < q0 + Qd) { kA[r - q0] = key; pA[r - q0] = pall[a]; }
+            }
+            cur = 0;
+            n = max(0, min(Qd, total - q0));
+            cluster.sync();
+        }
+    } else {
+        cluster.sync();
+    }
+    const int Q = ((total + CL - 1) / CL + 31) / 32 * 32;
+    const int bits = nrows <= 1 ? 0 : 32 - __clz(nrows - 1);
+    const int passes = sparse && total <= SPARSE_DIRECT ? 0 : (bits + RADIX_BITS - 1) / RADIX_BITS;
+    uint32_t* kst = reinterpret_cast<uint32_t*>(region);
+    uint16_t* pst = reinterpret_cast<uint16_t*>(kst + ST_QC);
+    uint16_t* rnk = pst + ST_QC;
+    const int d = threadIdx.x;
+    for (int ps = 0; ps < passes; ++ps) {
+        const int shift = ps * RADIX_BITS;
+        const int co = cur * ST_QC;
+        for (int i = threadIdx.x; i < ST_WARPS * RADIX / 2; i += ST_THREADS) reinterpret_cast<uint32_t*>(cnt)[i] = 0;
+        __syncthreads();
+        const int slots = (n + ST_THREADS - 1) / ST_THREADS;
+        const int wbase = warp * slots * 32;
+        for (int s = 0; s < slots; ++s) {
+            const int idx = wbase + s * 32 + lane;
+            const bool valid = idx < n;
+            const unsigned dg = valid ? ((kA[co + idx] >> shift) & (RADIX - 1)) : 0u;
+            const unsigned m = digit_peers(dg, valid);
+            const int leader = __ffs(m) - 1;
+            uint32_t old = 0;
+            if (valid && lane == leader) { old = cnt[warp * RADIX + dg]; cnt[warp * RADIX + dg] = (uint16_t)(old + __popc(m)); }
+            old = __shfl_sync(0xffffffffu, old, leader);
+            if (valid) rnk[idx] = (uint16_t)(old + __popc(m & lt));
+            __syncwarp();
+        }
+        __syncthreads();
+        {
+            uint32_t run = 0;
+            for (int w = 0; w < ST_WARPS; ++w) { const uint32_t t = cnt[w * RADIX + d]; cnt[w * RADIX + d] = (uint16_t)run; run += t; }
+            tot[d] = run;
+        }
+        __syncthreads();
+        if (warp == 0) {
+            uint32_t v[8], sum = 0;
+#pragma unroll
+            for (int j = 0; j < 8; ++j) { v[j] = tot[lane * 8 + j]; sum += v[j]; }
+            uint32_t inc = sum;
+#pragma unroll
+            for (int o = 1; o < 32; o <<= 1) { const uint32_t t = __shfl_up_sync(0xffffffffu, inc, o); if (lane >= o) inc += t; }
+            uint32_t ex = inc - sum;
+#pragma unroll
+            for (int j = 0; j < 8; ++j) { lstart[lane * 8 + j] = ex; ex += v[j]; }
+        }
+        __syncthreads();
+        for (int s = 0; s < slots; ++s) {
+            const int idx = wbase + s * 32 + lane;
+            if (idx < n) {
+                const uint32_t key = kA[co + idx];
+                const unsigned dg = (key >> shift) & (RADIX - 1);
+                const uint32_t lp = lstart[dg] + cnt[warp * RADIX + dg] + rnk[idx];
+                kst[lp] = key;
+                pst[lp] = pA[co + idx];
+            }
+        }
+        cluster.sync();
+        uint32_t before = 0;
+        {
+            uint32_t all = 0;
+#pragma unroll
+            for (int r = 0; r < CL; ++r) {
+                const uint32_t t = *cluster.map_shared_rank(&tot[d], r);
+                all += t;
+                if (r < crank) before += t;
+            }
+            base[d] = all;
+        }
+        __syncthreads();
+        if (warp == 0) {
+            uint32_t v[8], sum = 0;
+#pragma unroll
+            for (int j = 0; j < 8; ++j) { v[j] = base[lane * 8 + j]; sum += v[j]; }
+            uint32_t inc = sum;
+#pragma unroll
+            for (int o = 1; o < 32; o <<= 1) { const uint32_t t = __shfl_up_sync(0xffffffffu, inc, o); if (lane >= o) inc += t; }
+            uint32_t ex = inc - sum;
+#pragma unroll
+            for (int j = 0; j < 8; ++j) { base[lane * 8 + j] = ex; ex += v[j]; }
+        }
+        __syncthreads();
+        base[d] += before;
+        __syncthreads();
+        for (int i = threadIdx.x; i < n; i += ST_THREADS) {
+            const uint32_t kk = kst[i];
+            const unsigned dg = (kk >> shift) & (RADIX - 1);
+            const uint32_t pos = base[dg] + ((uint32_t)i - lstart[dg]);
+            const int dest = (int)(pos / (uint32_t)Q);
+            const uint32_t li = pos - (uint32_t)dest * (uint32_t)Q;
+            const uint32_t kaddr = (uint32_t)__cvta_generic_to_shared(st_smem) + 4u * (uint32_t)(ST_QC - co + (int)li);
+            const uint32_t paddr = (uint32_t)__cvta_generic_to_shared(st_smem) + 8u * ST_QC + 2u * (uint32_t)(ST_QC - co + (int)li);
+            uint32_t rk, rp;
+            asm("mapa.shared::cluster.u32 %0, %1, %2;" : "=r"(rk) : "r"(kaddr), "r"(dest));
+            asm("mapa.shared::cluster.u32 %0, %1, %2;" : "=r"(rp) : "r"(paddr), "r"(dest));
+            asm volatile("st.shared::cluster.u32 [%0], %1;" :: "r"(rk), "r"(kk) : "memory");
+            asm volatile("st.shared::cluster.u16 [%0], %1;" :: "r"(rp), "h"(pst[i]) : "memory");
+        }
+        cluster.sync();
+        cur ^= 1;
+        n = max(0, min(Q, total - crank * Q));
+    }
+    if (crank == 0) sort_stamp(sparse ? 16 + 8 * F + f : 16 + 4 * F + f);
+    const uint32_t* kc = kbuf(cur);
+    sort_tail<ST_THREADS>(kc, pbuf(cur), n, crank * Q, total, B, F, f, off, skeys, perm, posflag, rl_entries, rl_segc, rl_cap, F * CL_SEGS,
+                          f * CL_SEGS + crank, f * CL_SEGS + crank, [=](int gi) {
+        const int dest = gi / Q;
+        return *cg::this_cluster().map_shared_rank(kc + (gi - dest * Q), dest);
+    });
+    cluster.sync();
+    step_sort_event(crank ? -1 : 17 + (sparse ? 2 * F : 0) + 2 * f, true);
+    if (threadIdx.x == 0 && crank == 0 && sort_dbg()) {
+        unsigned long long* u = reinterpret_cast<unsigned long long*>(sort_dbg());
+        unsigned long long gt; asm volatile("mov.u64 %0, %globaltimer;" : "=l"(gt));
+        if (nrows > 100000u) atomicMin(u + 13, gt);
+        if (nrows <= 256u) atomicMax(u + 12, gt);
     }
 }
 
@@ -727,12 +816,21 @@
 }
 
 FMB_API int fmb_sort_fields_kernel_fns(const void** fns, int* nparams, int* skeys_arg) {
-    fns[0] = (const void*)sort_fields_kernel; nparams[0] = 11; skeys_arg[0] = 4;
-    fns[1] = (const void*)sort_fields_cluster_kernel<256, true, 16>; nparams[1] = 12; skeys_arg[1] = 4;
-    fns[2] = (const void*)sort_fields_cluster_kernel<1024, false, 16>; nparams[2] = 12; skeys_arg[2] = 4;
-    fns[3] = (const void*)sparse_fields_kernel; nparams[3] = 11; skeys_arg[3] = 5;
-    fns[4] = (const void*)sort_fields_cluster_kernel<256, true, 8>; nparams[4] = 12; skeys_arg[4] = 4;
+    fns[0] = (const void*)sort_fields_kernel; nparams[0] = 10; skeys_arg[0] = 4;
+    fns[1] = (const void*)sort_fields_cluster_kernel<256, true, 16>; nparams[1] = 11; skeys_arg[1] = 4;
+    fns[2] = (const void*)sort_fields_cluster_kernel<1024, false, 16>; nparams[2] = 11; skeys_arg[2] = 4;
+    fns[3] = (const void*)sort_fields_step_kernel; nparams[3] = 11; skeys_arg[3] = 4;
+    fns[4] = (const void*)sort_fields_cluster_kernel<256, true, 8>; nparams[4] = 11; skeys_arg[4] = 4;
     return 5;
+}
+
+FMB_API int fmb_sort_step_kernel_resources(int* out) {
+    cudaFuncAttributes a;
+    const cudaError_t e = cudaFuncGetAttributes(&a, sort_fields_step_kernel);
+    if (e != cudaSuccess) { fmb_set_error("cudaFuncGetAttributes: %s", cudaGetErrorString(e)); return FMB_ERR_CUDA; }
+    out[0] = a.numRegs; out[1] = (int)a.localSizeBytes; out[2] = (int)a.sharedSizeBytes;
+    out[3] = (int)ST_SMEM; out[4] = ST_THREADS; out[5] = CL;
+    return FMB_OK;
 }
 
 FMB_API int fmb_sort_fields_max_batch(void) { return 65536; }
@@ -748,11 +846,9 @@
 }
 
 FMB_API int64_t fmb_sort_fields_sparse_min_rows(int B) {
-    return (B > 0 && sparse_smem_bytes(B) <= 200 * 1024) ? (int64_t)16 * B : 0;
-}
-
-#define FMB_SORT_PART_DENSE 2
-#define FMB_SORT_PART_SPARSE 4
+    return (B > 0 && B <= ST_MAX_B) ? (int64_t)16 * B : 0;
+}
+
 FMB_API int fmb_sort_fields_ex(const int32_t* ids, int B, int F, const int32_t* field_off, int32_t* sorted_keys,
                                int32_t* perm, uint32_t* posflag, const fmb_runlist_t* rl, int flags, cudaStream_t stream) {
     FMB_CHECK_ARG(ids && field_off && sorted_keys && perm, "fmb_sort_fields: null pointer");
@@ -770,33 +866,28 @@
         cudaFuncSetAttribute(sort_fields_cluster_kernel<256, true, 8>, cudaFuncAttributeMaxDynamicSharedMemorySize, 220 * 1024);
         cudaFuncSetAttribute(sort_fields_cluster_kernel<256, true, 16>, cudaFuncAttributeMaxDynamicSharedMemorySize, 220 * 1024);
         cudaFuncSetAttribute(sort_fields_cluster_kernel<1024, false, 16>, cudaFuncAttributeMaxDynamicSharedMemorySize, 220 * 1024);
-        cudaFuncSetAttribute(sparse_fields_kernel, cudaFuncAttributeMaxDynamicSharedMemorySize, 220 * 1024);
+        cudaFuncSetAttribute(sort_fields_step_kernel, cudaFuncAttributeMaxDynamicSharedMemorySize, (int)ST_SMEM);
         attr = true;
     }
-    const bool sparse = (flags & FMB_SORT_SPARSE_OK) && posflag && fmb_sort_fields_sparse_min_rows(B) > 0;
-    const int64_t split = sparse ? fmb_sort_fields_sparse_min_rows(B) : ((int64_t)1 << 40);
-    const bool do_dense = !(flags & FMB_SORT_PART_SPARSE), do_sparse = sparse && !(flags & FMB_SORT_PART_DENSE);
-    if (!do_dense) {
+    if ((flags & FMB_SORT_SPARSE_OK) && posflag && fmb_sort_fields_sparse_min_rows(B) > 0) {
+        sort_fields_step_kernel<<<F * CL, ST_THREADS, ST_SMEM, stream>>>(
+            ids, B, F, field_off, sorted_keys, perm, fmb_sort_fields_sparse_min_rows(B), posflag, rle, rlc, rcap);
+        FMB_CHECK_LAUNCH("sort_fields_step_kernel");
     } else if (B <= 2048) {
         sort_fields_kernel<<<F, FS_THREADS, fmb::smem_sort_bytes(B), stream>>>(ids, B, F, field_off, sorted_keys, perm, posflag,
-                                                                               rle, rlc, rcap, split);
+                                                                               rle, rlc, rcap);
         FMB_CHECK_LAUNCH("sort_fields_kernel");
     } else {
         if (Bq <= 256 * 8)
             sort_fields_cluster_kernel<256, true, 8><<<F * CL, 256, fmb::smem_sort_bytes(Bq) + (size_t)Bq * 6 + 16, stream>>>(
-                ids, B, F, field_off, sorted_keys, perm, Bq, posflag, rle, rlc, rcap, split);
+                ids, B, F, field_off, sorted_keys, perm, Bq, posflag, rle, rlc, rcap);
         else if (Bq <= 256 * FS_MAX_SLOTS)
             sort_fields_cluster_kernel<256, true, 16><<<F * CL, 256, fmb::smem_sort_bytes(Bq) + (size_t)Bq * 6 + 16, stream>>>(
-                ids, B, F, field_off, sorted_keys, perm, Bq, posflag, rle, rlc, rcap, split);
+                ids, B, F, field_off, sorted_keys, perm, Bq, posflag, rle, rlc, rcap);
         else
             sort_fields_cluster_kernel<1024, false, 16><<<F * CL, 1024, fmb::smem_sort_bytes(Bq), stream>>>(
-                ids, B, F, field_off, sorted_keys, perm, Bq, posflag, rle, rlc, rcap, split);
+                ids, B, F, field_off, sorted_keys, perm, Bq, posflag, rle, rlc, rcap);
         FMB_CHECK_LAUNCH("sort_fields_cluster_kernel");
-    }
-    if (do_sparse) {
-        sparse_fields_kernel<<<F, SPARSE_THREADS, sparse_smem_bytes(B), stream>>>(ids, B, F, field_off, split, sorted_keys, perm,
-                                                                                   posflag, rle, rlc, rcap);
-        FMB_CHECK_LAUNCH("sparse_fields_kernel");
     }
     return FMB_OK;
 }
diff --git a/fm_for_online_recommendation_b200/csrc/session.cu b/fm_for_online_recommendation_b200/csrc/session.cu
--- a/fm_for_online_recommendation_b200/csrc/session.cu
+++ b/fm_for_online_recommendation_b200/csrc/session.cu
@@ -93,8 +93,8 @@
     cudaEvent_t ev_h2d[4], ev_done[4];
     int slot_used[4];
     int64_t launches;
-    cudaStream_t st0, st1, st2, st3, st4;
-    cudaEvent_t ev_sp_fork, ev_sp_join, ev_join4;
+    cudaStream_t st0, st1, st2, st4;
+    cudaEvent_t ev_join4;
     int64_t steps_done;
     cudaEvent_t ev_fork, ev_fwd, ev_sort, ev_join;
     int use_graph, use_prio;
@@ -125,9 +125,6 @@
     cudaFree(s->d_sort_ws2);
     if (s->ev_join2) cudaEventDestroy(s->ev_join2);
     for (int i = 0; i < s->npsg; ++i) if (s->psg[i].exec) { cudaGraphExecDestroy(s->psg[i].exec); cudaGraphDestroy(s->psg[i].graph); }
-    if (s->ev_sp_fork) cudaEventDestroy(s->ev_sp_fork);
-    if (s->ev_sp_join) cudaEventDestroy(s->ev_sp_join);
-    if (s->st3) cudaStreamDestroy(s->st3);
     if (s->st4) cudaStreamDestroy(s->st4);
     if (s->ev_join4) cudaEventDestroy(s->ev_join4);
     if (s->ev_presort) cudaEventDestroy(s->ev_presort);
@@ -198,11 +195,8 @@
         if (e == cudaSuccess) e = cudaStreamCreateWithPriority(&s->st0, cudaStreamNonBlocking, greatest);
         if (e == cudaSuccess) e = cudaStreamCreateWithPriority(&s->st1, cudaStreamNonBlocking, greatest);
         if (e == cudaSuccess) e = cudaStreamCreateWithPriority(&s->st2, cudaStreamNonBlocking, least);
-        if (e == cudaSuccess) e = cudaStreamCreateWithPriority(&s->st3, cudaStreamNonBlocking, least);
         if (e == cudaSuccess) e = cudaStreamCreateWithPriority(&s->st4, cudaStreamNonBlocking, greatest);
         if (e == cudaSuccess) e = cudaEventCreateWithFlags(&s->ev_join4, cudaEventDisableTiming);
-        if (e == cudaSuccess) e = cudaEventCreateWithFlags(&s->ev_sp_fork, cudaEventDisableTiming);
-        if (e == cudaSuccess) e = cudaEventCreateWithFlags(&s->ev_sp_join, cudaEventDisableTiming);
     }
     if (e == cudaSuccess) e = cudaEventCreateWithFlags(&s->ev_fork, cudaEventDisableTiming);
     if (e == cudaSuccess) e = cudaEventCreateWithFlags(&s->ev_fwd, cudaEventDisableTiming);
@@ -252,23 +246,9 @@
     rl.entries = s->d_runlist_buf[buf]; rl.seg_count = s->d_runcount_buf[buf];
     if (by_field_sort(s, B)) {
         fmb_runlist_shape(B, s->F, &rl.nseg, &rl.seg_cap);
-        if (!s->sparse_ok) {
-            *nlaunch += 1;
-            return fmb_sort_fields_ex(ids, B, s->F, s->d_field_off, s->d_skeys_buf[buf], s->d_perm_buf[buf],
-                                      s->d_posflag_buf[buf], &rl, 0, st);
-        }
-        cudaMemsetAsync(s->d_posflag_buf[buf], 0, (size_t)N * 4, st);
-        cudaEventRecord(s->ev_sp_fork, st);
-        cudaStreamWaitEvent(s->st3, s->ev_sp_fork, 0);
-        rc = fmb_sort_fields_ex(ids, B, s->F, s->d_field_off, s->d_skeys_buf[buf], s->d_perm_buf[buf], s->d_posflag_buf[buf],
-                                &rl, 1 | 2, st);
-        if (rc) return rc;
-        rc = fmb_sort_fields_ex(ids, B, s->F, s->d_field_off, s->d_skeys_buf[buf], s->d_perm_buf[buf], s->d_posflag_buf[buf],
-                                &rl, 1 | 4, s->st3);
-        cudaEventRecord(s->ev_sp_join, s->st3);
-        cudaStreamWaitEvent(st, s->ev_sp_join, 0);
-        *nlaunch += 2;
-        return rc;
+        *nlaunch += 1;
+        return fmb_sort_fields_ex(ids, B, s->F, s->d_field_off, s->d_skeys_buf[buf], s->d_perm_buf[buf],
+                                  s->d_posflag_buf[buf], &rl, s->sparse_ok , st);
     } else {
         rc = fmb_sort_segment(ids, N, key_bits, radix_ws, s->sort_ws_bytes, s->d_skeys_buf[buf], s->d_perm_buf[buf],
                               nullptr, nullptr, st);
```

Result: slower. 69.19 million, median of 6 (-65.8%).
